# tungphambasement/TNN

Hardware: AMD Instinct MI355X
Metric: images/sec (whole node) WRN-16-8 on 32x32x3, pipeline-parallel (higher is better)
Workload: dtype bf16; 1 GPU; model=cifar100_wrn16_8, global_batch=256, input=32x32x3, microbatches=1, graphed_step=True, parallelism=single

## Files before the change

tnn_amd/csrc/batchnorm.hip:

```cpp

#include "common.h"
#include "kernels.h"

namespace tnn {

template <typename T> struct alignas(16) BnPack {
  T e[16 / sizeof(T)];
};

template <typename T>
__global__ void k_bn_partial(const T* __restrict__ x, float* __restrict__ sum,
                             float* __restrict__ sumsq, int64_t rows,
                             int cols) {
  const int cpb = min(cols, 256);
  const int rows_per_iter = 256 / cpb;
  const int c = threadIdx.x % cpb + blockIdx.x * cpb;
  const int r_off = threadIdx.x / cpb;
  if (c >= cols || r_off >= rows_per_iter) return;
  const int64_t r0 = rows * blockIdx.y / gridDim.y;
  const int64_t r1 = rows * (blockIdx.y + 1) / gridDim.y;
  const float k = VecIO<T>::to_f32(x[c]);
  float s = 0.0f, ss = 0.0f;
  for (int64_t r = r0 + r_off; r < r1; r += rows_per_iter) {
    float v = VecIO<T>::to_f32(x[r * cols + c]) - k;
// ... 62 lines not shown
      ts += sh_s[(r * gpb + gl) * V + j];
      tss += sh_ss[(r * gpb + gl) * V + j];
    }
    int c = blockIdx.x * cpb_total + cl;
    if (c >= cols) break;
    sum[(int64_t)blockIdx.y * 2 * cols + c] = ts;
    sum[(int64_t)blockIdx.y * 2 * cols + cols + c] = tss;
  }
}

template <typename T>
__global__ void k_bn_bwd_reduce_vec(const T* __restrict__ x,
                                    const T* __restrict__ dy,
                                    const T* __restrict__ y_relu,
                                    const float* mean, const float* invstd,
                                    float* __restrict__ sum_dy,
                                    float* __restrict__ sum_dy_xhat,
                                    int64_t rows, int cols, float dy_scale) {
  constexpr int V = 16 / sizeof(T);
  using VecT = BnPack<T>;
  const int groups = cols / V;
  const int gpb = min(groups, 256);
  const int rows_per_iter = 256 / gpb;
  const int g = threadIdx.x % gpb + blockIdx.x * gpb;
  const int r_off = threadIdx.x / gpb;
  __shared__ float sh[2 * 256 * V];
  float* sh_s = sh;
  float* sh_sx = sh + 256 * V;
  float s[V] = {}, sx[V] = {};
  if (g < groups && r_off < rows_per_iter) {
    const int64_t r0 = rows * blockIdx.y / gridDim.y;
    const int64_t r1 = rows * (blockIdx.y + 1) / gridDim.y;
    float m[V], is[V];
#pragma unroll
    for (int j = 0; j < V; ++j) {
      m[j] = mean[g * V + j];
      is[j] = invstd[g * V + j];
    }
#pragma unroll 2
    for (int64_t r = r0 + r_off; r < r1; r += rows_per_iter) {
      int64_t i = r * cols + (int64_t)g * V;
      VecT vg = *(const VecT*)&dy[i];
      VecT vx = *(const VecT*)&x[i];
      if (y_relu) {
        VecT vy = *(const VecT*)&y_relu[i];
#pragma unroll
        for (int j = 0; j < V; ++j) {
          float gr = VecIO<T>::to_f32(vy.e[j]) > 0.0f
                         ? VecIO<T>::to_f32(vg.e[j]) * dy_scale : 0.0f;
          s[j] += gr;
          sx[j] += gr * (VecIO<T>::to_f32(vx.e[j]) - m[j]) * is[j];
        }
      } else {
#pragma unroll
        for (int j = 0; j < V; ++j) {
          float gr = VecIO<T>::to_f32(vg.e[j]) * dy_scale;
          s[j] += gr;
          sx[j] += gr * (VecIO<T>::to_f32(vx.e[j]) - m[j]) * is[j];
        }
      }
    }
  }
#pragma unroll
  for (int j = 0; j < V; ++j) {
    sh_s[threadIdx.x * V + j] = s[j];
    sh_sx[threadIdx.x * V + j] = sx[j];
  }
  __syncthreads();
  const int cpb_total = gpb * V;
  for (int cl = threadIdx.x; cl < cpb_total; cl += 256) {
    int gl = cl / V, j = cl % V;
    float ts = 0.0f, tsx = 0.0f;
    for (int r = 0; r < rows_per_iter; ++r) {
      ts += sh_s[(r * gpb + gl) * V + j];
      tsx += sh_sx[(r * gpb + gl) * V + j];
    }
    int c = blockIdx.x * cpb_total + cl;
    if (c >= cols) break;
    sum_dy[(int64_t)blockIdx.y * 2 * cols + c] = ts;
    sum_dy[(int64_t)blockIdx.y * 2 * cols + cols + c] = tsx;
  }
}

template <typename T>
__global__ void k_bn_finalize(float* mean, float* invstd, const float* sum,
                              const float* sumsq, const T* shift, float* rmean,
                              float* rvar, float momentum, int64_t rows,
                              int cols, float eps) {
  int c = blockIdx.x * blockDim.x + threadIdx.x;
  if (c >= cols) return;
  float d = sum[c] / rows;
  float var = fmaxf(sumsq[c] / rows - d * d, 0.0f);
  float m = shift ? VecIO<T>::to_f32(shift[c]) + d : d;
  mean[c] = m;
  invstd[c] = rsqrtf(var + eps);
  if (rmean) {
    float unbiased = var * ((float)rows / (float)(rows > 1 ? rows - 1 : 1));
    rmean[c] = rmean[c] * (1.0f - momentum) + m * momentum;
    rvar[c] = rvar[c] * (1.0f - momentum) + unbiased * momentum;
  }
}

template <typename T>
__global__ void k_bn_apply(const T* __restrict__ x, const float* mean,
                           const float* invstd, const float* gamma,
                           const float* beta, T* __restrict__ y, int64_t n,
                           int cols, bool relu) {
  int64_t i = (int64_t)blockIdx.x * blockDim.x + threadIdx.x;
  int64_t stride = (int64_t)gridDim.x * blockDim.x;
  for (; i < n; i += stride) {
    int c = i % cols;
    float v = (VecIO<T>::to_f32(x[i]) - mean[c]) * invstd[c] * gamma[c] + beta[c];
    if (relu) v = fmaxf(v, 0.0f);
    y[i] = VecIO<T>::from_f32(v);
  }
}

template <typename T>
__global__ void k_bn_apply_drop(const T* __restrict__ x, const float* mean,
                                const float* invstd, const float* gamma,
                                const float* beta, T* __restrict__ y,
                                int64_t n, int cols, float p, uint64_t seed,
                                const int64_t* __restrict__ ctr) {
  if (ctr) seed ^= (uint64_t)(*ctr) * 0x9E3779B97F4A7C15ull;
  const float scale = 1.0f / (1.0f - p);
  Philox rng(seed);
  int64_t i4 = (int64_t)blockIdx.x * blockDim.x + threadIdx.x;
  int64_t stride = (int64_t)gridDim.x * blockDim.x;
  for (; i4 * 4 < n; i4 += stride) {
    uint4 r = rng(i4);
    unsigned int rs[4] = {r.x, r.y, r.z, r.w};
#pragma unroll
    for (int j = 0; j < 4; ++j) {
      int64_t i = i4 * 4 + j;
      if (i < n) {
        int c = i % cols;
        float v =
            (VecIO<T>::to_f32(x[i]) - mean[c]) * invstd[c] * gamma[c] + beta[c];
        v = fmaxf(v, 0.0f);
        bool keep = u32_to_uniform(rs[j]) > p;
        y[i] = VecIO<T>::from_f32(keep ? v * scale : 0.0f);
      }
    }
  }
}

template <typename T>
__global__ void k_bn_apply_drop_vec(const T* __restrict__ x, const float* mean,
                                    const float* invstd, const float* gamma,
                                    const float* beta, T* __restrict__ y,
                                    int64_t nv, int groups, float p,
                                    uint64_t seed,
                                    const int64_t* __restrict__ ctr) {
  if (ctr) seed ^= (uint64_t)(*ctr) * 0x9E3779B97F4A7C15ull;
  constexpr int V = 16 / sizeof(T);
  using VecT = BnPack<T>;
  const float scale = 1.0f / (1.0f - p);
  Philox rng(seed);
  int64_t i = (int64_t)blockIdx.x * blockDim.x + threadIdx.x;
  int64_t stride = (int64_t)gridDim.x * blockDim.x;
  for (; i < nv; i += stride) {
    int c0 = (int)((uint32_t)i % (uint32_t)groups) * V;
    VecT vx = ((const VecT*)x)[i];
    uint4 r0 = rng(2 * i);
    uint4 r1 = rng(2 * i + 1);
    unsigned int rs[8] = {r0.x, r0.y, r0.z, r0.w, r1.x, r1.y, r1.z, r1.w};
    VecT vy;
#pragma unroll
    for (int j = 0; j < V; ++j) {
      int c = c0 + j;
      float v =
          (VecIO<T>::to_f32(vx.e[j]) - mean[c]) * invstd[c] * gamma[c] + beta[c];
      v = fmaxf(v, 0.0f);
      bool keep = u32_to_uniform(rs[j]) > p;
      vy.e[j] = VecIO<T>::from_f32(keep ? v * scale : 0.0f);
    }
    ((VecT*)y)[i] = vy;
  }
}

template <typename T>
__global__ void k_bn_infer(const T* __restrict__ x, const float* rmean,
                           const float* rvar, const float* gamma,
// ... 148 lines not shown
  int cblocks = (groups + gpb - 1) / gpb;
  int rows_per_iter = 256 / gpb;
  int64_t iters = (rows + rows_per_iter - 1) / rows_per_iter;
  int rslices = (int)std::min<int64_t>(std::max<int64_t>(512 / cblocks, 1),
                                       std::max<int64_t>(iters / 4, 1));
  return dim3(cblocks, rslices);
}

static inline dim3 bn_reduce_grid(int64_t rows, int cols) {
  int cpb = cols < 256 ? cols : 256;
  int cblocks = (cols + cpb - 1) / cpb;
  int rows_per_iter = 256 / cpb;
  int64_t iters = (rows + rows_per_iter - 1) / rows_per_iter;
  int rslices = (int)std::min<int64_t>(std::max<int64_t>(512 / cblocks, 1),
                                       std::max<int64_t>(iters / 4, 1));
  return dim3(cblocks, rslices);
}

int64_t bn_stats_ws_floats(DT dt, const void* x, int64_t rows, int cols) {
  const bool vec = dt == DT::F32 ? bn_vec_ok<float>((void*)x, cols)
                                 : bn_vec_ok<bf16>((void*)x, cols);
  if (!vec) return 0;
  dim3 g = dt == DT::F32 ? bn_reduce_grid_vec<float>(rows, cols)
                         : bn_reduce_grid_vec<bf16>(rows, cols);
  return ((int64_t)g.y + 1) * 2 * cols;
}

void bn_stats_launch(DT dt, const void* x, float* mean, float* invstd,
                     float* rmean, float* rvar, float momentum, float* ws,
                     int64_t rows, int cols, float eps, hipStream_t s) {
  if (ws) {
    dim3 g = dt == DT::F32 ? bn_reduce_grid_vec<float>(rows, cols)
                           : bn_reduce_grid_vec<bf16>(rows, cols);
    float* sums = ws + (int64_t)g.y * 2 * cols;
    if (dt == DT::F32)
      hipLaunchKernelGGL(k_bn_partial_vec<float>, g, dim3(256), 0, s,
                         (const float*)x, ws, nullptr, rows, cols);
    else
      hipLaunchKernelGGL(k_bn_partial_vec<bf16>, g, dim3(256), 0, s,
                         (const bf16*)x, ws, nullptr, rows, cols);
    slab_fin_launch(ws, sums, (int)g.y, 2 * cols, s);
    if (dt == DT::F32)
      hipLaunchKernelGGL(k_bn_finalize<float>, dim3((cols + 255) / 256),
                         dim3(256), 0, s, mean, invstd, sums, sums + cols,
                         (const float*)x, rmean, rvar, momentum, rows, cols,
                         eps);
    else
      hipLaunchKernelGGL(k_bn_finalize<bf16>, dim3((cols + 255) / 256),
                         dim3(256), 0, s, mean, invstd, sums, sums + cols,
                         (const bf16*)x, rmean, rvar, momentum, rows, cols,
                         eps);
    return;
  }
  hipMemsetAsync(mean, 0, cols * sizeof(float), s);
  hipMemsetAsync(invstd, 0, cols * sizeof(float), s);
  if (dt == DT::F32)
    hipLaunchKernelGGL(k_bn_partial<float>, bn_reduce_grid(rows, cols),
                       dim3(256), 0, s, (const float*)x, mean, invstd, rows,
                       cols);
  else
    hipLaunchKernelGGL(k_bn_partial<bf16>, bn_reduce_grid(rows, cols),
                       dim3(256), 0, s, (const bf16*)x, mean, invstd, rows,
                       cols);
  if (dt == DT::F32)
    hipLaunchKernelGGL(k_bn_finalize<float>, dim3((cols + 255) / 256),
                       dim3(256), 0, s, mean, invstd, mean, invstd,
                       (const float*)x, rmean, rvar, momentum, rows, cols, eps);
  else
    hipLaunchKernelGGL(k_bn_finalize<bf16>, dim3((cols + 255) / 256),
                       dim3(256), 0, s, mean, invstd, mean, invstd,
                       (const bf16*)x, rmean, rvar, momentum, rows, cols, eps);
}

void bn_finalize_launch(const float* sum, const float* sumsq, float* mean,
                        float* invstd, float* rmean, float* rvar,
                        float momentum, int64_t rows, int cols, float eps,
                        hipStream_t s) {
  hipLaunchKernelGGL(k_bn_finalize<float>, dim3((cols + 255) / 256),
                     dim3(256), 0, s, mean, invstd, sum, sumsq,
                     (const float*)nullptr, rmean, rvar, momentum, rows, cols,
                     eps);
}

void bn_apply_launch(DT dt, const void* x, const float* mean,
                     const float* invstd, const float* gamma, const float* beta,
                     void* y, int64_t rows, int cols, bool relu,
                     hipStream_t s) {
  int64_t n = rows * cols;
  int blocks = (int)std::min<int64_t>((n + 255) / 256, (int64_t)2048);
  if (dt == DT::F32) {
    if (bn_vec_ok<float>(x, cols)) {
      hipLaunchKernelGGL(k_bn_apply_vec<float>, dim3(blocks), dim3(256), 0, s,
                         (const float*)x, mean, invstd, gamma, beta, (float*)y,
                         n / 4, cols / 4, relu);
      return;
    }
    hipLaunchKernelGGL(k_bn_apply<float>, dim3(blocks), dim3(256), 0, s,
                       (const float*)x, mean, invstd, gamma, beta, (float*)y, n,
                       cols, relu);
  } else {
    if (bn_vec_ok<bf16>(x, cols)) {
      hipLaunchKernelGGL(k_bn_apply_vec<bf16>, dim3(blocks), dim3(256), 0, s,
                         (const bf16*)x, mean, invstd, gamma, beta, (bf16*)y,
                         n / 8, cols / 8, relu);
      return;
    }
    hipLaunchKernelGGL(k_bn_apply<bf16>, dim3(blocks), dim3(256), 0, s,
                       (const bf16*)x, mean, invstd, gamma, beta, (bf16*)y, n,
                       cols, relu);
  }
}

void bn_apply_drop_launch(DT dt, const void* x, const float* mean,
                          const float* invstd, const float* gamma,
                          const float* beta, void* y, int64_t rows, int cols,
                          float p, uint64_t seed, const int64_t* ctr,
                          hipStream_t s) {
  int64_t n = rows * cols;
  int V = dt == DT::F32 ? 4 : 8;
  if (cols % V == 0 && (((uintptr_t)x & 15) == 0) && n < (1ll << 34)) {
    int64_t nv = n / V;
    int blocks = (int)std::min<int64_t>((nv + 255) / 256, (int64_t)2048);
    if (dt == DT::F32)
      hipLaunchKernelGGL(k_bn_apply_drop_vec<float>, dim3(blocks), dim3(256),
                         0, s, (const float*)x, mean, invstd, gamma, beta,
                         (float*)y, nv, cols / V, p, seed, ctr);
    else
      hipLaunchKernelGGL(k_bn_apply_drop_vec<bf16>, dim3(blocks), dim3(256),
                         0, s, (const bf16*)x, mean, invstd, gamma, beta,
                         (bf16*)y, nv, cols / V, p, seed, ctr);
    return;
  }
  int blocks = (int)std::min<int64_t>(((n + 3) / 4 + 255) / 256, (int64_t)2048);
  if (dt == DT::F32)
    hipLaunchKernelGGL(k_bn_apply_drop<float>, dim3(blocks), dim3(256), 0, s,
                       (const float*)x, mean, invstd, gamma, beta, (float*)y, n,
                       cols, p, seed, ctr);
  else
    hipLaunchKernelGGL(k_bn_apply_drop<bf16>, dim3(blocks), dim3(256), 0, s,
                       (const bf16*)x, mean, invstd, gamma, beta, (bf16*)y, n,
                       cols, p, seed, ctr);
}

void bn_infer_launch(DT dt, const void* x, const float* rmean,
                     const float* rvar, const float* gamma, const float* beta,
                     void* y, int64_t rows, int cols, float eps, bool relu,
                     hipStream_t s) {
  int64_t n = rows * cols;
  int blocks = (int)std::min<int64_t>((n + 255) / 256, (int64_t)2048);
  if (dt == DT::F32)
    hipLaunchKernelGGL(k_bn_infer<float>, dim3(blocks), dim3(256), 0, s,
                       (const float*)x, rmean, rvar, gamma, beta, (float*)y, n,
                       cols, eps, relu);
  else
    hipLaunchKernelGGL(k_bn_infer<bf16>, dim3(blocks), dim3(256), 0, s,
                       (const bf16*)x, rmean, rvar, gamma, beta, (bf16*)y, n,
                       cols, eps, relu);
}

int64_t bn_bwd_ws_floats(DT dt, const void* x, const void* dy, int64_t rows,
                         int cols) {
  const bool vec = dt == DT::F32
                       ? (bn_vec_ok<float>((void*)x, cols) &&
                          bn_vec_ok<float>((void*)dy, cols))
                       : (bn_vec_ok<bf16>((void*)x, cols) &&
                          bn_vec_ok<bf16>((void*)dy, cols));
  if (!vec) return 0;
  dim3 g = dt == DT::F32 ? bn_reduce_grid_vec<float>(rows, cols)
                         : bn_reduce_grid_vec<bf16>(rows, cols);
  return (int64_t)g.y * 2 * cols;
}

void bn_bwd_reduce_launch(DT dt, const void* x, const void* dy,
                          const void* y_relu, const float* mean,
                          const float* invstd, float* sum_dy,
                          float* sum_dy_xhat, float* ws, int64_t rows,
                          int cols, float dy_scale, hipStream_t s) {
  if (ws) {
    dim3 g = dt == DT::F32 ? bn_reduce_grid_vec<float>(rows, cols)
                           : bn_reduce_grid_vec<bf16>(rows, cols);
    if (dt == DT::F32)
      hipLaunchKernelGGL(k_bn_bwd_reduce_vec<float>, g, dim3(256), 0, s,
                         (const float*)x, (const float*)dy,
                         (const float*)y_relu, mean, invstd, ws, nullptr,
                         rows, cols, dy_scale);
    else
      hipLaunchKernelGGL(k_bn_bwd_reduce_vec<bf16>, g, dim3(256), 0, s,
                         (const bf16*)x, (const bf16*)dy, (const bf16*)y_relu,
                         mean, invstd, ws, nullptr, rows, cols, dy_scale);
    slab_fin_launch(ws, sum_dy, (int)g.y, 2 * cols, s);
    return;
  }
  if (dt == DT::F32)
    hipLaunchKernelGGL(k_bn_bwd_reduce<float>, bn_reduce_grid(rows, cols),
                       dim3(256), 0, s, (const float*)x, (const float*)dy,
                       (const float*)y_relu, mean, invstd, sum_dy,
                       sum_dy_xhat, rows, cols, dy_scale);
  else
    hipLaunchKernelGGL(k_bn_bwd_reduce<bf16>, bn_reduce_grid(rows, cols),
                       dim3(256), 0, s, (const bf16*)x, (const bf16*)dy,
                       (const bf16*)y_relu, mean, invstd, sum_dy,
                       sum_dy_xhat, rows, cols, dy_scale);
}

void bn_bwd_apply_launch(DT dt, const void* x, const void* dy,
                         const void* y_relu, const float* mean,
                         const float* invstd, const float* gamma,
                         const float* sum_dy, const float* sum_dy_xhat,
                         void* dx, const void* resid, int64_t rows, int cols,
                         float dy_scale, hipStream_t s) {
  int64_t n = rows * cols;
  int blocks = (int)std::min<int64_t>((n + 255) / 256, (int64_t)2048);
  const bool vec = dt == DT::F32 ? bn_vec_ok<float>(x, cols)
                                 : bn_vec_ok<bf16>(x, cols);
  if (dt == DT::F32) {
    if (vec && ((uintptr_t)dy & 15) == 0) {
      hipLaunchKernelGGL(k_bn_bwd_apply_vec<float>, dim3(blocks), dim3(256),
                         0, s, (const float*)x, (const float*)dy,
                         (const float*)y_relu, mean, invstd, gamma, sum_dy,
                         sum_dy_xhat, (float*)dx, (const float*)resid,
                         n / 4, cols / 4, rows, dy_scale);
      return;
    }
    hipLaunchKernelGGL(k_bn_bwd_apply<float>, dim3(blocks), dim3(256), 0, s,
                       (const float*)x, (const float*)dy, (const float*)y_relu,
                       mean, invstd, gamma, sum_dy, sum_dy_xhat, (float*)dx,
                       (const float*)resid, n, rows, cols, dy_scale);
  } else {
    if (vec && ((uintptr_t)dy & 15) == 0) {
      hipLaunchKernelGGL(k_bn_bwd_apply_vec<bf16>, dim3(blocks), dim3(256),
                         0, s, (const bf16*)x, (const bf16*)dy,
                         (const bf16*)y_relu, mean, invstd, gamma, sum_dy,
                         sum_dy_xhat, (bf16*)dx, (const bf16*)resid,
                         n / 8, cols / 8, rows, dy_scale);
      return;
    }
    hipLaunchKernelGGL(k_bn_bwd_apply<bf16>, dim3(blocks), dim3(256), 0, s,
                       (const bf16*)x, (const bf16*)dy, (const bf16*)y_relu,
                       mean, invstd, gamma, sum_dy, sum_dy_xhat, (bf16*)dx,
                       (const bf16*)resid, n, rows, cols, dy_scale);
  }
}

}
```

tnn_amd/csrc/bindings.cpp:

```cpp

#include <array>
#include <torch/extension.h>
#include <ATen/hip/HIPContext.h>

#include "kernels.h"

namespace tnn {

static hipStream_t cur_stream() {
  return at::hip::getCurrentHIPStreamMasqueradingAsCUDA().stream();
}

static void* zero_page(const at::Tensor& like) {
  static at::Tensor z;
  if (!z.defined() || z.device() != like.device())
    z = at::zeros({16}, like.options().dtype(at::kFloat));
  return z.data_ptr();
}

static DT dt_of(const at::Tensor& t) {
  if (t.scalar_type() == at::kFloat) return DT::F32;
  if (t.scalar_type() == at::kBFloat16) return DT::BF16;
  TORCH_CHECK(false, "tnn_amd kernels support fp32/bf16, got ", t.scalar_type());
}
// ... 394 lines not shown
  int64_t H = x.size(1), W = x.size(2);
  return conv_shape_out(fn, x.size(0), H, W, Cin, Cout, KH, KW, SH, SW, PH, PW,
                        conv_out_extent(H, KH, SH, PH),
                        conv_out_extent(W, KW, SW, PW));
}

static ConvShape conv_fwd_shape(const char* fn, const at::Tensor& x,
                                const at::Tensor& w, int64_t sh, int64_t sw,
                                int64_t ph, int64_t pw) {
  CHECK_IN(x);
  CHECK_IN(w);
  TORCH_CHECK(x.dim() == 4 && w.dim() == 4 && x.size(3) == w.size(2), fn,
              " x ", x.sizes(), " w ", w.sizes());
  TORCH_CHECK(x.scalar_type() == w.scalar_type(), fn, " dtype mismatch ",
              x.scalar_type(), " vs ", w.scalar_type());
  return conv_shape(fn, x, w.size(2), w.size(3), w.size(0), w.size(1), sh, sw,
                    ph, pw);
}

static ConvShape conv_dgrad_shape(const char* fn, const at::Tensor& dy,
                                  const at::Tensor& w, int64_t H, int64_t W,
                                  int64_t sh, int64_t sw, int64_t ph,
                                  int64_t pw) {
  CHECK_IN(dy);
  CHECK_IN(w);
  TORCH_CHECK(dy.dim() == 4 && w.dim() == 4, fn, " dy ", dy.sizes(), " w ",
              w.sizes());
  TORCH_CHECK(dy.scalar_type() == w.scalar_type(), fn,
              " dtype mismatch: dy is ", dy.scalar_type(), ", w is ",
              w.scalar_type());
  TORCH_CHECK(dy.size(3) == w.size(3), fn, " dy ", dy.sizes(),
              " has other channels than w ", w.sizes());
  const int64_t KH = w.size(0), KW = w.size(1);
  auto cs = conv_shape_out(fn, dy.size(0), H, W, w.size(2), w.size(3), KH, KW,
                           sh, sw, ph, pw, conv_out_extent(H, KH, sh, ph),
                           conv_out_extent(W, KW, sw, pw));
  TORCH_CHECK(dy.size(1) == cs.OH && dy.size(2) == cs.OW, fn, " dy ",
              dy.sizes(), " is not the output of a ", H, " x ", W,
              " input: expected OH = ", cs.OH, ", OW = ", cs.OW);
  return cs;
}

static ConvShape conv_wgrad_shape(const char* fn, const at::Tensor& x,
                                  const at::Tensor& dy, int64_t KH, int64_t KW,
                                  int64_t sh, int64_t sw, int64_t ph,
                                  int64_t pw) {
  CHECK_IN(x);
  CHECK_IN(dy);
  TORCH_CHECK(x.dim() == 4 && dy.dim() == 4, fn, " x ", x.sizes(), " dy ",
              dy.sizes());
  TORCH_CHECK(x.scalar_type() == dy.scalar_type(), fn,
              " dtype mismatch: x is ", x.scalar_type(), ", dy is ",
              dy.scalar_type());
  TORCH_CHECK(x.size(0) == dy.size(0), fn, " batch mismatch: x ", x.sizes(),
              " dy ", dy.sizes());
  auto cs = conv_shape(fn, x, x.size(3), dy.size(3), KH, KW, sh, sw, ph, pw);
  TORCH_CHECK(dy.size(1) == cs.OH && dy.size(2) == cs.OW, "wgrad shape");
  return cs;
}

static std::vector<at::Tensor> conv2d_fwd_impl(
    const at::Tensor& x, const at::Tensor& w,
    const c10::optional<at::Tensor>& bias, int64_t sh, int64_t sw, int64_t ph,
    int64_t pw, bool relu, bool want_stats) {
  auto cs = conv_fwd_shape("conv2d_fwd", x, w, sh, sw, ph, pw);
  if (bias.has_value()) {
    TORCH_CHECK(bias->scalar_type() == x.scalar_type(),
                "conv2d bias dtype mismatch");
    TORCH_CHECK(bias->is_cuda() && bias->is_contiguous() &&
                    bias->numel() == cs.Cout,
                "conv2d_fwd: bias must be a contiguous GPU tensor of ",
                cs.Cout, " elements, got ", bias->sizes());
  }
  auto y = at::empty({cs.N, cs.OH, cs.OW, cs.Cout}, x.options());
  at::Tensor wt2, stats;
  const bool db = conv2d_fwd_wants_db(dt_of(x), x.data_ptr(), cs);
  if (db) {
    wt2 = at::empty({(int64_t)cs.Cout, (int64_t)cs.KH * cs.KW * cs.Cin},
                    w.options());
    transpose_w_fwd_launch(dt_of(x), w.data_ptr(), wt2.data_ptr(),
                           cs.KH * cs.KW, cs.Cin, cs.Cout, cur_stream());
  }
  if (want_stats)
    stats = db ? at::zeros({2, (int64_t)cs.Cout},
                           x.options().dtype(at::kFloat))
               : at::empty({0}, x.options().dtype(at::kFloat));
  conv2d_fwd_launch(dt_of(x), x.data_ptr(), w.data_ptr(),
                    db ? wt2.data_ptr() : nullptr,
                    bias.has_value() ? bias->data_ptr() : nullptr,
                    y.data_ptr(), zero_page(x),
                    db && want_stats ? stats.data_ptr<float>() : nullptr, cs,
                    relu, cur_stream());
  return {y, stats};
}

at::Tensor conv2d_fwd(const at::Tensor& x, const at::Tensor& w,
                      const c10::optional<at::Tensor>& bias, int64_t sh,
                      int64_t sw, int64_t ph, int64_t pw, bool relu) {
  return conv2d_fwd_impl(x, w, bias, sh, sw, ph, pw, relu, false)[0];
}

std::vector<at::Tensor> conv2d_fwd_stats(const at::Tensor& x,
                                         const at::Tensor& w,
                                         const c10::optional<at::Tensor>& bias,
                                         int64_t sh, int64_t sw, int64_t ph,
                                         int64_t pw) {
  return conv2d_fwd_impl(x, w, bias, sh, sw, ph, pw, false, true);
}

at::Tensor conv2d_dgrad(const at::Tensor& dy, const at::Tensor& w, int64_t H,
                        int64_t W, int64_t sh, int64_t sw, int64_t ph,
                        int64_t pw) {
  auto cs = conv_dgrad_shape("conv2d_dgrad", dy, w, H, W, sh, sw, ph, pw);
  int KH = cs.KH, KW = cs.KW, Cin = cs.Cin, Cout = cs.Cout;
  auto dx = at::empty({cs.N, H, W, Cin}, dy.options());
  if (conv2d_dgrad_wants_db(dt_of(dy), dy.data_ptr(), cs)) {
    auto w_t2d = at::empty({Cin, (int64_t)KH * KW * Cout}, w.options());
    transpose_w_dgrad_launch(dt_of(w), w.data_ptr(), w_t2d.data_ptr(), KH * KW,
                             Cin, Cout, cur_stream());
    conv2d_dgrad_launch(dt_of(dy), dy.data_ptr(), nullptr, w_t2d.data_ptr(),
                        dx.data_ptr(), zero_page(dy), cs, cur_stream());
    return dx;
  }
  auto w_t = at::empty({KH, KW, Cout, Cin}, w.options());
  transpose_w_launch(dt_of(w), w.data_ptr(), w_t.data_ptr(), KH, KW, Cin, Cout,
                     cur_stream());
  conv2d_dgrad_launch(dt_of(dy), dy.data_ptr(), w_t.data_ptr(), nullptr,
                      dx.data_ptr(), zero_page(dy), cs, cur_stream());
  return dx;
}

std::string conv2d_fwd_route_name(const at::Tensor& x, const at::Tensor& w,
                                  int64_t sh, int64_t sw, int64_t ph,
                                  int64_t pw, bool stats) {
  auto cs = conv_fwd_shape("conv2d_fwd_route", x, w, sh, sw, ph, pw);
  return conv2d_fwd_route(dt_of(x), x.data_ptr(), cs, stats);
}

std::string conv2d_dgrad_route_name(const at::Tensor& dy,
                                    const at::Tensor& w, int64_t H, int64_t W,
                                    int64_t sh, int64_t sw, int64_t ph,
                                    int64_t pw) {
  auto cs = conv_dgrad_shape("conv2d_dgrad_route", dy, w, H, W, sh, sw, ph,
                             pw);
  return conv2d_dgrad_route(dt_of(dy), dy.data_ptr(), cs);
}

std::tuple<std::string, int64_t> conv2d_wgrad_route_name(
    const at::Tensor& x, const at::Tensor& dy, int64_t KH, int64_t KW,
    int64_t sh, int64_t sw, int64_t ph, int64_t pw) {
  auto cs = conv_wgrad_shape("conv2d_wgrad_route", x, dy, KH, KW, sh, sw, ph,
                             pw);
  return {conv2d_wgrad_route(dt_of(x), x.data_ptr(), dy.data_ptr(), cs),
          conv2d_wgrad_zsplits(dt_of(x), x.data_ptr(), dy.data_ptr(), cs)};
}

static at::Tensor conv2d_wgrad_rows(const at::Tensor& x, const at::Tensor& dy,
                                    int64_t KH, int64_t KW, int64_t sh,
                                    int64_t sw, int64_t ph, int64_t pw,
                                    bool out_in_dt, bool bias) {
  auto cs = conv_wgrad_shape("conv2d_wgrad", x, dy, KH, KW, sh, sw, ph, pw);
  DT out_dt = out_in_dt ? dt_of(x) : DT::F32;
  const int64_t rows = KH * KW * cs.Cin + (bias ? 1 : 0);
  auto out = at::empty({rows, (int64_t)cs.Cout},
                       out_dt == DT::F32 ? x.options().dtype(at::kFloat)
                                         : x.options());
  int z = conv2d_wgrad_zsplits(dt_of(x), x.data_ptr(), dy.data_ptr(), cs);
  at::Tensor ws;
  float* wsp = nullptr;
  if (z > 1 || out_dt != DT::F32) {
    ws = at::empty({(int64_t)z * rows * cs.Cout},
                   x.options().dtype(at::kFloat));
    wsp = ws.data_ptr<float>();
  }
  conv2d_wgrad_launch(dt_of(x), x.data_ptr(), dy.data_ptr(), out.data_ptr(),
                      out_dt, wsp, z, zero_page(x), cs, bias, cur_stream());
  return out;
}

at::Tensor conv2d_wgrad(const at::Tensor& x, const at::Tensor& dy, int64_t KH,
                        int64_t KW, int64_t sh, int64_t sw, int64_t ph,
                        int64_t pw, bool out_in_dt) {
  return conv2d_wgrad_rows(x, dy, KH, KW, sh, sw, ph, pw, out_in_dt, false)
      .view({KH, KW, x.size(3), dy.size(3)});
}

std::vector<at::Tensor> conv2d_wgrad_bias(const at::Tensor& x,
                                          const at::Tensor& dy, int64_t KH,
                                          int64_t KW, int64_t sh, int64_t sw,
                                          int64_t ph, int64_t pw,
                                          bool out_in_dt) {
  auto out = conv2d_wgrad_rows(x, dy, KH, KW, sh, sw, ph, pw, out_in_dt, true);
  const int64_t kout = out.size(0) - 1;
  return {out.narrow(0, 0, kout).view({KH, KW, x.size(3), dy.size(3)}),
          out.select(0, kout)};
}

std::vector<at::Tensor> bn_fwd_train(const at::Tensor& x,
                                     const at::Tensor& gamma,
                                     const at::Tensor& beta,
                                     const c10::optional<at::Tensor>& rmean,
                                     const c10::optional<at::Tensor>& rvar,
                                     double momentum, double eps, bool relu,
                                     double dropout_p, int64_t seed,
                                     const c10::optional<at::Tensor>& precomp,
                                     const c10::optional<at::Tensor>& ctr =
                                         c10::nullopt) {
  CHECK_IN(x);
  TORCH_CHECK(dropout_p == 0.0 || relu, "fused BN dropout requires relu");
  int C = x.size(-1);
  int64_t rows = x.numel() / C;
  auto mean = at::empty({C}, x.options().dtype(at::kFloat));
  auto invstd = at::empty({C}, x.options().dtype(at::kFloat));
  auto y = at::empty_like(x);
  float* rm = rmean.has_value() ? rmean->data_ptr<float>() : nullptr;
  float* rv = rvar.has_value() ? rvar->data_ptr<float>() : nullptr;
  if (precomp.has_value()) {
    TORCH_CHECK(precomp->numel() == 2 * C, "bad precomputed stats");
    const float* ps = precomp->data_ptr<float>();
    bn_finalize_launch(ps, ps + C, mean.data_ptr<float>(),
                       invstd.data_ptr<float>(), rm, rv, (float)momentum,
                       rows, C, (float)eps, cur_stream());
  } else {
    const int64_t wsn = bn_stats_ws_floats(dt_of(x), x.data_ptr(), rows, C);
    at::Tensor ws;
    float* wp = nullptr;
    if (wsn) {
      ws = at::empty({wsn}, x.options().dtype(at::kFloat));
      wp = ws.data_ptr<float>();
    }
    bn_stats_launch(dt_of(x), x.data_ptr(), mean.data_ptr<float>(),
                    invstd.data_ptr<float>(), rm, rv, (float)momentum, wp,
                    rows, C, (float)eps, cur_stream());
  }
  if (dropout_p > 0.0)
    bn_apply_drop_launch(dt_of(x), x.data_ptr(), mean.data_ptr<float>(),
                         invstd.data_ptr<float>(), gamma.data_ptr<float>(),
                         beta.data_ptr<float>(), y.data_ptr(), rows, C,
                         (float)dropout_p, (uint64_t)seed,
                         ctr.has_value() ? ctr->data_ptr<int64_t>() : nullptr,
                         cur_stream());
  else
    bn_apply_launch(dt_of(x), x.data_ptr(), mean.data_ptr<float>(),
                    invstd.data_ptr<float>(), gamma.data_ptr<float>(),
                    beta.data_ptr<float>(), y.data_ptr(), rows, C, relu,
                    cur_stream());
  return {y, mean, invstd};
}

at::Tensor bn_fwd_infer(const at::Tensor& x, const at::Tensor& gamma,
                        const at::Tensor& beta, const at::Tensor& rmean,
                        const at::Tensor& rvar, double eps, bool relu) {
  CHECK_IN(x);
  int C = x.size(-1);
  int64_t rows = x.numel() / C;
  auto y = at::empty_like(x);
  bn_infer_launch(dt_of(x), x.data_ptr(), rmean.data_ptr<float>(),
                  rvar.data_ptr<float>(), gamma.data_ptr<float>(),
                  beta.data_ptr<float>(), y.data_ptr(), rows, C, (float)eps,
                  relu, cur_stream());
  return y;
}

std::vector<at::Tensor> bn_bwd(const at::Tensor& x, const at::Tensor& dy,
                               const at::Tensor& gamma, const at::Tensor& mean,
                               const at::Tensor& invstd,
                               const c10::optional<at::Tensor>& y_relu,
                               double dy_scale,
                               const c10::optional<at::Tensor>& resid =
                                   c10::nullopt) {
  CHECK_IN(x);
  CHECK_IN(dy);
  const void* resp = nullptr;
  if (resid.has_value()) {
    TORCH_CHECK(resid->is_contiguous() &&
                resid->scalar_type() == x.scalar_type() &&
                resid->numel() == x.numel(), "bn_bwd resid mismatch");
    resp = resid->data_ptr();
  }
  int C = x.size(-1);
  int64_t rows = x.numel() / C;
  const int64_t wsn = bn_bwd_ws_floats(dt_of(x), x.data_ptr(),
                                       dy.data_ptr(), rows, C);
  auto sums = wsn ? at::empty({2, C}, x.options().dtype(at::kFloat))
                  : at::zeros({2, C}, x.options().dtype(at::kFloat));
  auto sum_dy = sums[0];
  auto sum_dy_xhat = sums[1];
  at::Tensor ws;
  float* wp = nullptr;
  if (wsn) {
    ws = at::empty({wsn}, x.options().dtype(at::kFloat));
    wp = ws.data_ptr<float>();
  }
  auto dx = at::empty_like(x);
  const void* yr = y_relu.has_value() ? y_relu->data_ptr() : nullptr;
  bn_bwd_reduce_launch(dt_of(x), x.data_ptr(), dy.data_ptr(), yr,
                       mean.data_ptr<float>(), invstd.data_ptr<float>(),
                       sum_dy.data_ptr<float>(), sum_dy_xhat.data_ptr<float>(),
                       wp, rows, C, (float)dy_scale, cur_stream());
  bn_bwd_apply_launch(dt_of(x), x.data_ptr(), dy.data_ptr(), yr,
                      mean.data_ptr<float>(), invstd.data_ptr<float>(),
                      gamma.data_ptr<float>(), sum_dy.data_ptr<float>(),
                      sum_dy_xhat.data_ptr<float>(), dx.data_ptr(), resp,
                      rows, C, (float)dy_scale, cur_stream());
  return {dx, sum_dy_xhat, sum_dy};
}

static PoolShape pool_shape(const at::Tensor& x, int KH, int KW, int SH, int SW,
                            int PH, int PW) {
  PoolShape ps;
  ps.N = x.size(0);
  ps.H = x.size(1);
  ps.W = x.size(2);
  ps.C = x.size(3);
  ps.KH = KH;
  ps.KW = KW;
  ps.SH = SH;
  ps.SW = SW;
  ps.PH = PH;
  ps.PW = PW;
  ps.OH = (ps.H + 2 * PH - KH) / SH + 1;
  ps.OW = (ps.W + 2 * PW - KW) / SW + 1;
  return ps;
}

std::vector<at::Tensor> maxpool_fwd(const at::Tensor& x, int64_t kh, int64_t kw,
                                    int64_t sh, int64_t sw, int64_t ph,
                                    int64_t pw) {
  CHECK_IN(x);
  auto ps = pool_shape(x, kh, kw, sh, sw, ph, pw);
  auto y = at::empty({ps.N, ps.OH, ps.OW, ps.C}, x.options());
  auto idx = at::empty({ps.N, ps.OH, ps.OW, ps.C}, x.options().dtype(at::kInt));
  maxpool_fwd_launch(dt_of(x), x.data_ptr(), y.data_ptr(), idx.data_ptr<int>(),
                     ps, cur_stream());
  return {y, idx};
}

at::Tensor maxpool_bwd(const at::Tensor& dy, const at::Tensor& idx, int64_t H,
                       int64_t W) {
  CHECK_IN(dy);
  PoolShape ps;
  ps.N = dy.size(0);
  ps.OH = dy.size(1);
  ps.OW = dy.size(2);
  ps.C = dy.size(3);
  ps.H = H;
  ps.W = W;
  auto dxf = at::zeros({ps.N, H, W, ps.C}, dy.options().dtype(at::kFloat));
  maxpool_bwd_launch(dt_of(dy), dy.data_ptr(), idx.data_ptr<int>(),
                     dxf.data_ptr<float>(), ps, cur_stream());
  if (dy.scalar_type() == at::kFloat) return dxf;
  auto dx = at::empty({ps.N, H, W, ps.C}, dy.options());
  cast_f32_launch(dt_of(dy), dxf.data_ptr<float>(), dx.data_ptr(), dx.numel(),
                  cur_stream());
  return dx;
}

at::Tensor avgpool_fwd(const at::Tensor& x, int64_t kh, int64_t kw, int64_t sh,
                       int64_t sw, int64_t ph, int64_t pw) {
  CHECK_IN(x);
  auto ps = pool_shape(x, kh, kw, sh, sw, ph, pw);
  auto y = at::empty({ps.N, ps.OH, ps.OW, ps.C}, x.options());
  avgpool_fwd_launch(dt_of(x), x.data_ptr(), y.data_ptr(), ps, cur_stream());
  return y;
}

at::Tensor avgpool_bwd(const at::Tensor& dy, int64_t H, int64_t W, int64_t kh,
                       int64_t kw, int64_t sh, int64_t sw, int64_t ph,
                       int64_t pw) {
  CHECK_IN(dy);
  PoolShape ps;
  ps.N = dy.size(0);
  ps.OH = dy.size(1);
  ps.OW = dy.size(2);
  ps.C = dy.size(3);
  ps.H = H;
  ps.W = W;
  ps.KH = kh;
  ps.KW = kw;
  ps.SH = sh;
  ps.SW = sw;
  ps.PH = ph;
  ps.PW = pw;
  auto dx = at::empty({ps.N, H, W, ps.C}, dy.options());
  avgpool_bwd_launch(dt_of(dy), dy.data_ptr(), dx.data_ptr(), ps, cur_stream());
  return dx;
}

// ... 577 lines not shown
                cap = k_cache.size(2), D = k_cache.size(3);
  const int64_t T = k_new.size(2);
  const int64_t per = 16 / k_cache.element_size();
  auto vec_ok = [&](const at::Tensor& t) {
    return ((uintptr_t)t.data_ptr() & 15) == 0 && t.stride(0) % per == 0 &&
           t.stride(1) % per == 0 && t.stride(2) % per == 0;
  };
  const bool vec = D % per == 0 && vec_ok(k_new) && vec_ok(v_new) &&
                   vec_ok(k_cache) && vec_ok(v_cache);
  const std::array<int64_t, 3> ks = {k_new.stride(0), k_new.stride(1),
                                     k_new.stride(2)};
  const std::array<int64_t, 3> vs = {v_new.stride(0), v_new.stride(1),
                                     v_new.stride(2)};
  kv_append_n_launch(dt, k_cache.data_ptr(), v_cache.data_ptr(),
                     k_new.data_ptr(), v_new.data_ptr(),
                     pos.data_ptr<int64_t>(),
                     n_new.has_value() ? n_new->data_ptr<int64_t>() : nullptr,
                     (int)B, (int)H, (int)T, (int)cap, (int)D, ks.data(),
                     vs.data(), vec, cur_stream());
}

at::Tensor sample_logits(const at::Tensor& logits, double temperature,
                         int64_t top_k, double top_p, int64_t seed,
                         const at::Tensor& step,
                         const c10::optional<at::Tensor>& u) {
  CHECK_IN(logits);
  TORCH_CHECK(logits.dim() == 2 && logits.scalar_type() == at::kBFloat16,
              "sample_logits wants bf16 [R,V] logits");
  const int64_t R = logits.size(0), V = logits.size(1);
  TORCH_CHECK(V >= 1 && V < (int64_t)1 << 31, "sample_logits: bad V ", V);
  TORCH_CHECK(temperature >= 0.0 && top_k >= 0 && top_p > 0.0 && top_p <= 1.0,
              "sample_logits wants temperature >= 0, top_k >= 0, top_p in "
              "(0, 1]");
  TORCH_CHECK(step.is_cuda() && step.scalar_type() == at::kLong &&
              step.numel() == 1, "sample_logits step must be int64 [1]");
  const float* up = nullptr;
  if (u.has_value()) {
    TORCH_CHECK(u->is_cuda() && u->is_contiguous() &&
                u->scalar_type() == at::kFloat && u->numel() == R,
                "sample_logits u must be fp32 [R] on device");
    up = u->data_ptr<float>();
  }
  auto ids = at::empty({R}, logits.options().dtype(at::kLong));
  if (R > 0)
    sample_logits_launch(logits.data_ptr(), ids.data_ptr<int64_t>(), (int)R,
                         (int)V, (float)temperature,
                         (int)std::min<int64_t>(top_k, V), (float)top_p,
                         (uint64_t)seed, step.data_ptr<int64_t>(), up,
                         cur_stream());
  return ids;
}

namespace imgcodec {
at::Tensor decode_image(const py::bytes& data);
}

}

PYBIND11_MODULE(TORCH_EXTENSION_NAME, m) {
  m.def("act_fwd", &tnn::act_fwd);
  m.def("act_bwd", &tnn::act_bwd);
  m.def("relu_bwd_mask", &tnn::relu_bwd_mask);
  m.def("add_act_fwd", &tnn::add_act_fwd);
  m.def("add_act_bwd", &tnn::add_act_bwd);
  m.def("dropout_fwd", &tnn::dropout_fwd, py::arg("x"), py::arg("p"),
        py::arg("seed"), py::arg("ctr") = c10::nullopt);
  m.def("dropout_bwd", &tnn::dropout_bwd);
  m.def("colsum", &tnn::colsum);
  m.def("gemm", &tnn::gemm, py::arg("a"), py::arg("b"), py::arg("bias"),
        py::arg("act_kind"), py::arg("residual") = c10::nullopt,
        py::arg("ln_gamma") = c10::nullopt, py::arg("ln_beta") = c10::nullopt,
        py::arg("ln_eps") = 1e-5);
  m.def("gemm_skinny", &tnn::gemm_skinny, py::arg("a"), py::arg("b"),
        py::arg("bias"), py::arg("act_kind"),
        py::arg("residual") = c10::nullopt, py::arg("ln_gamma") = c10::nullopt,
        py::arg("ln_beta") = c10::nullopt, py::arg("ln_eps") = 1e-5);
  m.def("skinny_enabled", &tnn::skinny_enabled);
  m.def("gemm_nt", &tnn::gemm_nt);
  m.def("gemm_tn", &tnn::gemm_tn);
  m.def("mfma_selftest", &tnn::mfma_selftest);
  m.def("mfma_selftest_f32", &tnn::mfma_selftest_f32);
  m.def("conv2d_fwd", &tnn::conv2d_fwd);
  m.def("conv2d_fwd_stats", &tnn::conv2d_fwd_stats);
  m.def("conv2d_dgrad", &tnn::conv2d_dgrad);
  m.def("conv2d_fwd_route", &tnn::conv2d_fwd_route_name);
  m.def("conv2d_dgrad_route", &tnn::conv2d_dgrad_route_name);
  m.def("conv2d_wgrad_route", &tnn::conv2d_wgrad_route_name);
  m.def("conv2d_wgrad", &tnn::conv2d_wgrad);
  m.def("conv2d_wgrad_bias", &tnn::conv2d_wgrad_bias);
  m.def("bn_fwd_train", &tnn::bn_fwd_train, py::arg("x"), py::arg("gamma"),
        py::arg("beta"), py::arg("rmean"), py::arg("rvar"),
        py::arg("momentum"), py::arg("eps"), py::arg("relu"),
        py::arg("dropout_p"), py::arg("seed"), py::arg("precomp"),
        py::arg("ctr") = c10::nullopt);
  m.def("bn_fwd_infer", &tnn::bn_fwd_infer);
  m.def("bn_bwd", &tnn::bn_bwd, py::arg("x"), py::arg("dy"),
        py::arg("gamma"), py::arg("mean"), py::arg("invstd"),
        py::arg("y_relu"), py::arg("dy_scale"),
        py::arg("resid") = py::none());
  m.def("maxpool_fwd", &tnn::maxpool_fwd);
  m.def("maxpool_bwd", &tnn::maxpool_bwd);
  m.def("avgpool_fwd", &tnn::avgpool_fwd);
  m.def("avgpool_bwd", &tnn::avgpool_bwd);
  m.def("ce_fwd", &tnn::ce_fwd);
  m.def("ce_bwd", &tnn::ce_bwd);
  m.def("ptloss_fwd", &tnn::ptloss_fwd);
  m.def("ptloss_bwd", &tnn::ptloss_bwd);
  m.def("gn_fwd", &tnn::gn_fwd);
  m.def("gn_bwd", &tnn::gn_bwd);
  m.def("ln_fwd", &tnn::ln_fwd);
  m.def("ln_bwd", &tnn::ln_bwd, py::arg("x"), py::arg("dy"),
        py::arg("gamma"), py::arg("mean"), py::arg("invstd"),
        py::arg("resid") = py::none());
  m.def("embedding_fwd", &tnn::embedding_fwd);
  m.def("embedding_bwd", &tnn::embedding_bwd);
  m.def("attn_fwd", &tnn::attn_fwd);
  m.def("attn_bwd", &tnn::attn_bwd, py::arg("q"), py::arg("k"),
        py::arg("v"), py::arg("o"), py::arg("dout"), py::arg("lse"),
        py::arg("causal"), py::arg("dq_out") = py::none(),
        py::arg("dk_out") = py::none(), py::arg("dv_out") = py::none());
  m.def("bmm", &tnn::bmm);
  m.def("smax_fwd", &tnn::smax_fwd);
  m.def("smax_bwd", &tnn::smax_bwd);
  m.def("attn_decode", &tnn::attn_decode);
  m.def("kv_append", &tnn::kv_append);
  m.def("attn_extend", &tnn::attn_extend);
  m.def("kv_append_n", &tnn::kv_append_n);
  m.def("sample_logits", &tnn::sample_logits, py::arg("logits"),
        py::arg("temperature"), py::arg("top_k"), py::arg("top_p"),
        py::arg("seed"), py::arg("step"), py::arg("u") = c10::nullopt);
  m.def("sgd_step", &tnn::sgd_step, py::arg("param"), py::arg("master"),
        py::arg("grad"), py::arg("momentum_buf"), py::arg("lr"),
        py::arg("momentum"), py::arg("weight_decay"), py::arg("nesterov"),
        py::arg("clip") = c10::nullopt, py::arg("lr_dev") = c10::nullopt);
  m.def("adam_step", &tnn::adam_step, py::arg("param"), py::arg("master"),
        py::arg("grad"), py::arg("m"), py::arg("v"), py::arg("step"),
        py::arg("lr"), py::arg("beta1"), py::arg("beta2"), py::arg("eps"),
        py::arg("weight_decay"), py::arg("adamw"),
        py::arg("step_dev") = c10::nullopt, py::arg("clip") = c10::nullopt,
        py::arg("lr_dev") = c10::nullopt);
  m.def("adam_step_mt", &tnn::adam_step_mt, py::arg("desc"),
        py::arg("chunks"), py::arg("dt_p"), py::arg("dt_g"),
        py::arg("has_master"), py::arg("step"), py::arg("lr"),
        py::arg("beta1"), py::arg("beta2"), py::arg("eps"),
        py::arg("weight_decay"), py::arg("adamw"),
        py::arg("step_dev") = c10::nullopt, py::arg("clip") = c10::nullopt,
        py::arg("lr_dev") = c10::nullopt);
  m.def("grad_sumsq_mt", &tnn::grad_sumsq_mt, py::arg("desc"),
        py::arg("chunks"), py::arg("stride"), py::arg("gslot"),
        py::arg("nslot"), py::arg("dt_g"), py::arg("part"), py::arg("base"));
  m.def("clip_finalize", &tnn::clip_finalize, py::arg("part"),
        py::arg("npart"), py::arg("max_norm"), py::arg("state"),
        py::arg("skipped") = c10::nullopt, py::arg("sumsq_in") = c10::nullopt);
  m.def("decode_image", &tnn::imgcodec::decode_image);
}
```

tnn_amd/csrc/conv2d.hip:

```cpp

#include "common.h"
#include "kernels.h"
#include "tile_gemm.h"

namespace tnn {

using namespace tile;

template <bool POW2>
DEV int idiv(int x, const IDiv& f) {
  if constexpr (POW2) return x >> f.lg;
  else if (f.magic)
    return (int)(((unsigned long long)(unsigned)x * f.magic) >> f.sh);
  else
    return x / f.d;
}
template <bool POW2>
DEV int imod(int x, const IDiv& f) {
  if constexpr (POW2) return x & (f.d - 1);
  else return x - idiv<POW2>(x, f) * f.d;
}

DEV void kdecode(int kidx, const ConvShape& cs, int& kh, int& kw) {
  kh = (kidx * cs.mkw16) >> 16;
// ... 89 lines not shown
    int rem = row - n * (Hc * Wc);
    ih = idiv<POW2>(rem, cs.d_w);
    iw = rem - ih * Wc;
    if constexpr (S2) {
      ih = 2 * ih + cls_a;
      iw = 2 * iw + cls_b;
    }
  }
  template <bool POW2>
  DEV int64_t pixel(const ConvShape& cs, int row) const {
    if constexpr (!S2) return row;
    int n, ih, iw;
    coords<POW2>(cs, row, n, ih, iw);
    return ((int64_t)n * cs.H + ih) * cs.W + iw;
  }
};
template <bool S2, bool S1, typename T>
DEV const T* dgrad_src(const T* __restrict__ DY, const ConvShape& cs, int n,
                       int ih, int iw, int kh, int kw, int co, const T* oob) {
  int th = ih + cs.PH - kh, tw = iw + cs.PW - kw;
  int oh, ow;
  if constexpr (S2) {
    if (th < 0 || tw < 0) return oob;
    oh = th >> 1, ow = tw >> 1;
    if (oh >= cs.OH || ow >= cs.OW) return oob;
  } else if constexpr (S1) {
    if (th < 0 || tw < 0 || th >= cs.OH || tw >= cs.OW) return oob;
    oh = th, ow = tw;
  } else {
    if (th < 0 || tw < 0 || th % cs.SH || tw % cs.SW) return oob;
    oh = th / cs.SH, ow = tw / cs.SW;
    if (oh >= cs.OH || ow >= cs.OW) return oob;
  }
  return &DY[(((int64_t)n * cs.OH + oh) * cs.OW + ow) * cs.Cout + co];
}

template <typename T, typename GatherFn>
DEV void stage_a_gathered(T* As, int m0, int k0, int M, int K,
                          GatherFn&& gather) {
  constexpr int V = 16 / sizeof(T);
#pragma unroll
  for (int c = threadIdx.x; c < BM * (BK / V); c += THREADS) {
    int row = c / (BK / V);
    int kk = (c % (BK / V)) * V;
    int gm = m0 + row, gk = k0 + kk;
    Pack16<T> v = {};
    if (gm < M && gk < K) v = gather(gm, gk);
    *(Pack16<T>*)&As[lds_off<T>(row, kk)] = v;
  }
}
template <typename T, typename RowFn>
DEV void stage_b_transposed(T* Bs, RowFn&& rowptr, int ncols, int n0, int k0,
                            int K) {
  constexpr int V = 16 / sizeof(T);
#pragma unroll
  for (int c = threadIdx.x; c < BK * (BN / V); c += THREADS) {
    int kk = c / (BN / V);
    int nn = (c % (BN / V)) * V;
    int gk = k0 + kk;
    Pack16<T> v = {};
    if (gk < K) v = load16_guarded(rowptr(gk), n0 + nn, ncols);
#pragma unroll
    for (int j = 0; j < V; ++j)
      Bs[lds_off<T>(nn + j, kk)] = v.e[j];
  }
}


template <typename T, typename S>
DEV void conv_fwd_store(const WaveCoordT<S>& wc, f32x4 acc[S::FM][S::FN],
                        const T* bias, T* Y, const ConvShape& cs, int act_kind,
                        int m0, int n0, int M) {
  epilogue_visit(wc, acc, m0, n0, [&](int row, int col, float v) {
    if (row < M && col < cs.Cout) {
      if (bias) v += VecIO<T>::to_f32(bias[col]);
      if (act_kind != ACT_LINEAR) v = act_apply(v, act_kind);
      Y[(int64_t)row * cs.Cout + col] = VecIO<T>::from_f32(v);
    }
  });
}

template <typename T, typename S>
DEV void conv_fwd_stats(const WaveCoordT<S>& wc, f32x4 acc[S::FM][S::FN],
                        const T* bias_p, float* stats, const ConvShape& cs,
                        int m0, int n0, int M) {
  constexpr int FM = S::FM, FN = S::FN;
  float* ssum = stats;
  float* ssumsq = stats + cs.Cout;
  const int cr = (wc.lane >> 4) * 4;
  const int cc = wc.lane & 15;
#pragma unroll
  for (int fn = 0; fn < FN; ++fn) {
    int col = n0 + wc.wcol0 + fn * 16 + cc;
    float bias = 0.0f;
    if (col < cs.Cout) {
      if (bias_p) bias = VecIO<T>::to_f32(bias_p[col]);
    }
    float s = 0.0f, ss = 0.0f;
#pragma unroll
    for (int fm = 0; fm < FM; ++fm)
#pragma unroll
      for (int j = 0; j < 4; ++j) {
        int row = m0 + wc.wrow0 + fm * 16 + cr + j;
        if (row < M && col < cs.Cout) {
          float v = acc[fm][fn][j] + bias;
          s += v;
          ss += v * v;
        }
      }
    s += __shfl_xor(s, 16, 64);
    ss += __shfl_xor(ss, 16, 64);
    s += __shfl_xor(s, 32, 64);
    ss += __shfl_xor(ss, 32, 64);
    if (wc.lane < 16 && col < cs.Cout) {
      atomicAdd(&ssum[col], s);
      atomicAdd(&ssumsq[col], ss);
    }
  }
}

template <bool POW2, typename T, bool S2, typename S>
DEV void dgrad_store(const WaveCoordT<S>& wc, f32x4 acc[S::FM][S::FN], T* DX,
                     const ConvShape& cs, const DgradClass<S2>& dc, int m0,
                     int n0) {
  epilogue_visit(wc, acc, m0, n0, [&](int row, int col, float v) {
    if (row < dc.M && col < cs.Cin)
      DX[dc.template pixel<POW2>(cs, row) * cs.Cin + col] =
          VecIO<T>::from_f32(v);
  });
}

template <typename S>
DEV float* wgrad_slab_store(const WaveCoordT<S>& wc,
                            f32x4 acc[S::FM][S::FN], float* DW,
                            const ConvShape& cs, int Kout, int bias_row,
                            int r0, int n0) {
  float* out = DW + (int64_t)blockIdx.z * (Kout + bias_row) * cs.Cout;
  epilogue_visit(wc, acc, r0, n0, [&](int row, int col, float v) {
    if (row < Kout && col < cs.Cout) out[(int64_t)row * cs.Cout + col] = v;
  });
  return out;
}
template <typename S>
DEV void wgrad_biasrow_store(float* out, const WaveCoordT<S>& wc,
                             const f32x4 (&bacc)[S::FN / S::WAVES_M],
                             const ConvShape& cs, int Kout, int n0) {
  constexpr int NBF = S::FN / S::WAVES_M;
  const int wm = wc.wid / S::WAVES_N;
  if (wc.lane < 16) {
#pragma unroll
    for (int t = 0; t < NBF; ++t) {
      int col = n0 + wc.wcol0 + 16 * (NBF * wm + t) + wc.lane;
      if (col < cs.Cout) out[(int64_t)Kout * cs.Cout + col] = bacc[t][0];
    }
  }
}
DEV void wgrad_colsum_store(float* out, const ConvShape& cs, int Kout, int n0,
                            float bsum) {
  bsum = colsum_tile_finish(bsum);
  int col = n0 + (threadIdx.x >> 2);
  if ((threadIdx.x & 3) == 0 && col < cs.Cout)
    out[(int64_t)Kout * cs.Cout + col] = bsum;
}

template <bool DB, typename T, typename S, typename RowFn, typename TapFn,
          typename AtFn>
DEV void conv_db_kloop(T* As0, T* As1, T* Bs0, T* Bs1,
                       const WaveCoordT<S>& wc, f32x4 acc[S::FM][S::FN],
                       const T* __restrict__ asrc, int lgSW, int lgC,
                       const T* __restrict__ bsrc, int64_t bstride,
                       int brows, int m0, int n0, int K,
                       const T* __restrict__ zero16, RowFn&& row,
                       TapFn&& tap, AtFn&& at) {
  constexpr int NA = glds_count<T, S::BM>();
  constexpr int NB = glds_count<T, S::BN>();
  constexpr int NPER = NA + NB;
  const int wid = __builtin_amdgcn_readfirstlane(wc.wid);
  const bool uni = lgC >= 6;

  const T* ab[NA];
  int ap[NA], aq[NA];
  const T* bb[NB];
  bool bok[NB];
#pragma unroll
  for (int i = 0; i < NA; ++i) {
    const int j = wid * NA + i;
    int64_t noff;
    int p, q;
    const bool ok = row(m0 + glds_row<T>(j, wc.lane), noff, p, q);
    ab[i] = asrc + noff + (uni ? glds_kk<T>(j, wc.lane) : 0);
    ap[i] = ok ? p : -(1 << 28);
    aq[i] = q;
  }
#pragma unroll
  for (int i = 0; i < NB; ++i) {
    const int j = wid * NB + i;
    const int gn = n0 + glds_row<T>(j, wc.lane);
    bok[i] = gn < brows;
    bb[i] = bsrc + (int64_t)gn * bstride + (uni ? glds_kk<T>(j, wc.lane) : 0);
  }
// ... 43 lines not shown
  const int nch = (K + BK - 1) / BK;
  if (nch == 0) return;
  auto compute = [&](const T* a_img, const T* b_img) {
    if constexpr (sizeof(T) == 2)
      mfma_compute_tile_nofence(a_img, b_img, wc, acc);
    else
      mfma_compute_tile(a_img, b_img, wc, acc);
  };
  auto step = [&](int t, T* a_cur, T* b_cur, T* a_nxt, T* b_nxt) {
    if (t + 1 < nch) {
      stage(t + 1, a_nxt, b_nxt);
      wait_vmcnt<NPER>();
    } else {
      wait_vmcnt<0>();
    }
    __builtin_amdgcn_s_barrier();
    compute(a_cur, b_cur);
    __builtin_amdgcn_s_barrier();
  };
  if constexpr (DB) {
    stage(0, As0, Bs0);
    for (int t = 0; t < nch; t += 2) {
      step(t, As0, Bs0, As1, Bs1);
      if (t + 1 < nch) step(t + 1, As1, Bs1, As0, Bs0);
    }
  } else {
    for (int t = 0; t < nch; ++t) {
      stage(t, As0, Bs0);
      wait_vmcnt<0>();
      __builtin_amdgcn_s_barrier();
      compute(As0, Bs0);
      __builtin_amdgcn_s_barrier();
    }
  }
}

template <typename T, bool STATS, bool DB, typename S = TileStd>
DEV void conv_fwd_glds_tile(const T* __restrict__ X,
                            const T* __restrict__ WT2,
                            const T* __restrict__ bias, T* __restrict__ Y,
                            const T* __restrict__ zero16, const ConvShape& cs,
                            int act_kind, float* __restrict__ stats) {
  const int M = cs.N * cs.OH * cs.OW;
  const int K = cs.KH * cs.KW * cs.Cin;
  int tm_, tn_;
  conv_tile_order(cs, tm_, tn_);
  const int m0 = tm_ * S::BM;
  const int n0 = tn_ * S::BN;
  const WaveCoordT<S> wc;
  f32x4 acc[S::FM][S::FN] = {};

  auto row = [&](int gm, int64_t& noff, int& p, int& q) {
    const int n = gm >> cs.d_ohow.lg;
    const int rem = gm & (cs.OH * cs.OW - 1);
    p = (rem >> cs.d_ow.lg) * cs.SH - cs.PH;
    q = (rem & (cs.OW - 1)) * cs.SW - cs.PW;
    noff = (int64_t)n << (cs.d_hw.lg + cs.d_cin.lg);
    return gm < M;
  };
  auto tap = [&](int gk, int& dh, int& dw, int& c, int& bcol) {
    kdecode(gk >> cs.d_cin.lg, cs, dh, dw);
    c = gk & (cs.Cin - 1);
    bcol = gk;
  };
  auto at = [&](int p, int q, int dh, int dw, int& ih, int& iw) {
    ih = p + dh;
    iw = q + dw;
    return (unsigned)ih < (unsigned)cs.H && (unsigned)iw < (unsigned)cs.W;
  };
  if constexpr (DB) {
    __shared__ alignas(16) T As0[S::BM * BK], As1[S::BM * BK];
    __shared__ alignas(16) T Bs0[S::BN * BK], Bs1[S::BN * BK];
    conv_db_kloop<true>(As0, As1, Bs0, Bs1, wc, acc, X, cs.d_w.lg,
                        cs.d_cin.lg, WT2, (int64_t)K, cs.Cout, m0, n0, K,
                        zero16, row, tap, at);
  } else {
    __shared__ alignas(16) T As0[S::BM * BK], Bs0[S::BN * BK];
    conv_db_kloop<false>(As0, As0, Bs0, Bs0, wc, acc, X, cs.d_w.lg,
                         cs.d_cin.lg, WT2, (int64_t)K, cs.Cout, m0, n0, K,
                         zero16, row, tap, at);
  }

  conv_fwd_store(wc, acc, bias, Y, cs, act_kind, m0, n0, M);
  if constexpr (STATS) conv_fwd_stats(wc, acc, bias, stats, cs, m0, n0, M);
}

template <typename T, bool STATS = false>
__launch_bounds__(THREADS)
__global__ void k_conv_fwd_db(const T* __restrict__ X,
                              const T* __restrict__ WT2,
                              const T* __restrict__ bias, T* __restrict__ Y,
                              const T* __restrict__ zero16, ConvShape cs,
                              int act_kind, float* __restrict__ stats) {
  conv_fwd_glds_tile<T, STATS, true>(X, WT2, bias, Y, zero16, cs, act_kind,
                                     stats);
}

template <bool STATS>
__launch_bounds__(THREADS)
__global__ void k_conv_fwd_sb(const bf16* __restrict__ X,
                              const bf16* __restrict__ WT2,
                              const bf16* __restrict__ bias,
                              bf16* __restrict__ Y,
                              const bf16* __restrict__ zero16, ConvShape cs,
                              int act_kind, float* __restrict__ stats) {
  conv_fwd_glds_tile<bf16, STATS, false>(X, WT2, bias, Y, zero16, cs, act_kind,
                                         stats);
}

template <bool STATS>
__launch_bounds__(THREADS, 2)
__global__ void k_conv_fwd_db_wide(const bf16* __restrict__ X,
                                   const bf16* __restrict__ WT2,
                                   const bf16* __restrict__ bias,
                                   bf16* __restrict__ Y,
                                   const bf16* __restrict__ zero16,
                                   ConvShape cs, int act_kind,
                                   float* __restrict__ stats) {
  conv_fwd_glds_tile<bf16, STATS, true, TileWide>(X, WT2, bias, Y, zero16, cs,
                                                  act_kind, stats);
}
template <bool STATS>
__launch_bounds__(THREADS, 3)
__global__ void k_conv_fwd_sb_wide(const bf16* __restrict__ X,
                                   const bf16* __restrict__ WT2,
                                   const bf16* __restrict__ bias,
                                   bf16* __restrict__ Y,
                                   const bf16* __restrict__ zero16,
                                   ConvShape cs, int act_kind,
                                   float* __restrict__ stats) {
  conv_fwd_glds_tile<bf16, STATS, false, TileWide>(X, WT2, bias, Y, zero16, cs,
                                                   act_kind, stats);
}

template <typename T, bool POW2, bool GLDS>
__launch_bounds__(THREADS)
__global__ void k_conv_fwd(const T* __restrict__ X, const T* __restrict__ Wt,
                           const T* __restrict__ bias, T* __restrict__ Y,
                           const T* __restrict__ zero16, ConvShape cs,
                           int act_kind) {
  static_assert(!GLDS || POW2, "the LDS-DMA gate implies an all-pow2 shape");
  __shared__ alignas(16) T As[BM * BK];
  __shared__ alignas(16) T Bs[BN * BK];

  const int M = cs.N * cs.OH * cs.OW;
  const int K = cs.KH * cs.KW * cs.Cin;
  int tm_, tn_;
  conv_tile_order(cs, tm_, tn_);
  const int m0 = tm_ * BM;
  const int n0 = tn_ * BN;
  const WaveCoord wc;
  f32x4 acc[FM][FN] = {};

  auto a_src = [&](int k0, int rl, int kk) -> const T* {
    int gm = m0 + rl, gk = k0 + kk;
    if (gm >= M || gk >= K) return zero16;
    return fwd_src<POW2>(X, cs, fwd_row<POW2>(cs, gm), gk, zero16);
  };

  for (int k0 = 0; k0 < K; k0 += BK) {
    if constexpr (GLDS) {
      glds_stage_a<T>(As, wc, [&](int rl, int kk) { return a_src(k0, rl, kk); });
    } else {
      stage_a_gathered(As, m0, k0, M, K, [&](int gm, int gk) {
        return fwd_gather16<POW2>(X, cs, fwd_row<POW2>(cs, gm), gk, K);
      });
    }
// ... 462 lines not shown
                                    T* __restrict__ out, int rows, int cols) {
  __shared__ T tile[32][33];
  const int c0 = blockIdx.x * 32, r0 = blockIdx.y * 32;
  const int64_t slice = (int64_t)blockIdx.z * rows * cols;
  const T* src = in + slice;
  T* dst = out + slice;
  const int tx = threadIdx.x & 31, ty = threadIdx.x >> 5;
#pragma unroll
  for (int d = 0; d < 32; d += 8) {
    int r = r0 + ty + d, c = c0 + tx;
    if (r < rows && c < cols) tile[ty + d][tx] = src[(int64_t)r * cols + c];
  }
  __syncthreads();
#pragma unroll
  for (int d = 0; d < 32; d += 8) {
    int c = c0 + ty + d, r = r0 + tx;
    if (c < cols && r < rows) dst[(int64_t)c * rows + r] = tile[tx][ty + d];
  }
}

template <typename T>
__global__ void k_transpose_w_dgrad(const T* __restrict__ W,
                                    T* __restrict__ WT2D, int KHW, int Cin,
                                    int Cout) {
  int64_t i = (int64_t)blockIdx.x * blockDim.x + threadIdx.x;
  int64_t n = (int64_t)KHW * Cin * Cout;
  if (i >= n) return;
  int co = i % Cout;
  int ci = (i / Cout) % Cin;
  int64_t khw = i / ((int64_t)Cin * Cout);
  WT2D[((int64_t)ci * KHW + khw) * Cout + co] = W[i];
}

template <typename T>
__global__ void k_transpose_w_dgrad_vec(const T* __restrict__ W,
                                        T* __restrict__ WT2D, int KHW,
                                        int Cin, int Cout) {
  constexpr int V = 16 / sizeof(T);
  struct alignas(16) P { T e[16 / sizeof(T)]; };
  const int cov = Cout / V;
  int64_t i = (int64_t)blockIdx.x * blockDim.x + threadIdx.x;
  int64_t n = (int64_t)KHW * Cin * cov;
  if (i >= n) return;
  int c = i % cov;
  int ci = (i / cov) % Cin;
  int64_t khw = i / ((int64_t)Cin * cov);
  ((P*)WT2D)[((int64_t)ci * KHW + khw) * cov + c] =
      ((const P*)W)[((int64_t)khw * Cin + ci) * cov + c];
}

static bool all_pow2(const ConvShape& cs) {
  return cs.d_ohow.lg >= 0 && cs.d_ow.lg >= 0 && cs.d_cin.lg >= 0 &&
         cs.d_hw.lg >= 0 && cs.d_w.lg >= 0 && cs.d_cout.lg >= 0;
}

static bool vec_ok(DT dt, const void* ptr, int channels) {
  return channels % vec_elems(dt) == 0 && ptr_aligned16(ptr);
}

static int env_int(const char* name, int dflt) {
  const char* e = getenv(name);
  return e ? atoi(e) : dflt;
}

static bool db_on() {
  static const bool on = env_int("TNN_FWD_DB", 1) != 0;
  return on;
}

static int fwd_db_maxk() {
  static const int maxk = env_int("TNN_DB_MAXK", 2304);
  return maxk;
}

static int wide_mode() {
  static const int mode = env_int("TNN_CONV_WIDE", 1);
  return mode;
}
static int wide_buf() {
  static const int buf = env_int("TNN_CONV_WIDE_BUF", 0);
  return buf;
}

enum class Wide { NO, DB, SB };
constexpr int WIDE_MIN_TILES = 512;
constexpr int WIDE_FWD_DB_MINK = 2048;
constexpr int WIDE_DGRAD_SB_MAXK = 1152;
static Wide wide_pick(bool eligible, int tiles, bool take, bool single) {
  if (!eligible || wide_mode() == 0) return Wide::NO;
  if (wide_mode() == 1 && !(take && tiles >= WIDE_MIN_TILES)) return Wide::NO;
  if (wide_buf() != 0) single = wide_buf() == 2;
  return single ? Wide::SB : Wide::DB;
}
static Wide fwd_wide(DT dt, bool have_wt2, const ConvShape& cs, bool stats) {
  const int nt = cs.Cout / TileWide::BN;
  const int K = cs.KH * cs.KW * cs.Cin;
  const bool take = nt == 1 ? !stats : K >= WIDE_FWD_DB_MINK;
  return wide_pick(
      have_wt2 && dt == DT::BF16 && cs.Cout % TileWide::BN == 0,
      ceil_div(cs.N * cs.OH * cs.OW, TileWide::BM) * nt, take, nt == 1);
}
static Wide dgrad_wide(DT dt, bool have_wt2d, bool s2, const ConvShape& cs) {
  const int M = s2 ? cs.N * (cs.H / 2) * (cs.W / 2) : cs.N * cs.H * cs.W;
  const int taps =
      s2 ? ((cs.KH + 1) / 2) * ((cs.KW + 1) / 2) : cs.KH * cs.KW;
  return wide_pick(
      have_wt2d && dt == DT::BF16 && cs.Cin % TileWide::BN == 0,
      ceil_div(M, TileWide::BM) * (cs.Cin / TileWide::BN) * (s2 ? 4 : 1),
      true, taps * cs.Cout <= WIDE_DGRAD_SB_MAXK);
}

template <typename... KArgs, typename... Args>
static void launch(void (*kern)(KArgs...), dim3 grid, hipStream_t s,
                   Args... args) {
  hipLaunchKernelGGL(kern, grid, dim3(THREADS), 0, s, args...);
}

bool conv2d_fwd_wants_db(DT dt, const void* x, const ConvShape& cs) {
  if (!db_on()) return false;
  if (dt == DT::F32 && cs.KH * cs.KW * cs.Cin > fwd_db_maxk()) return false;
  return all_pow2(cs) && vec_ok(dt, x, cs.Cin);
}

static void transpose2d_launch(DT dt, const void* in, void* out, int batch,
                               int rows, int cols, hipStream_t s) {
  dim3 grid((cols + 31) / 32, (rows + 31) / 32, batch);
  dispatch_dt(dt, [&](auto tag) {
    using T = typename decltype(tag)::type;
    hipLaunchKernelGGL(k_transpose2d_tiled<T>, grid, dim3(256), 0, s,
                       (const T*)in, (T*)out, rows, cols);
  });
}

void transpose_w_fwd_launch(DT dt, const void* w, void* w_t2, int KHW, int Cin,
                            int Cout, hipStream_t s) {
  transpose2d_launch(dt, w, w_t2, 1, KHW * Cin, Cout, s);
}

void transpose_w_launch(DT dt, const void* w, void* w_t, int KH, int KW,
                        int Cin, int Cout, hipStream_t s) {
  transpose2d_launch(dt, w, w_t, KH * KW, Cin, Cout, s);
}

void transpose_w_dgrad_launch(DT dt, const void* w, void* w_t2d, int KHW,
                              int Cin, int Cout, hipStream_t s) {
  const bool vec = vec_ok(dt, w, Cout);
  int64_t n = (int64_t)KHW * Cin * (vec ? Cout / vec_elems(dt) : Cout);
  int blocks = (int)((n + 255) / 256);
  dispatch_dt(dt, [&](auto tag) {
    using T = typename decltype(tag)::type;
    auto kern = vec ? k_transpose_w_dgrad_vec<T> : k_transpose_w_dgrad<T>;
    hipLaunchKernelGGL(kern, dim3(blocks), dim3(256), 0, s, (const T*)w,
                       (T*)w_t2d, KHW, Cin, Cout);
  });
}

enum class FwdRoute { SB_WIDE, DB_WIDE, SB, DB, GLDS, POW2, GENERIC };
static FwdRoute fwd_route(DT dt, const void* x, bool have_wt2,
                          const ConvShape& cs, bool stats) {
  if (have_wt2) {
    const Wide wide = fwd_wide(dt, true, cs, stats);
    if (wide != Wide::NO)
      return wide == Wide::SB ? FwdRoute::SB_WIDE : FwdRoute::DB_WIDE;
    const bool long_k =
        dt == DT::BF16 && cs.KH * cs.KW * cs.Cin > fwd_db_maxk();
    return long_k ? FwdRoute::SB : FwdRoute::DB;
  }
  if (!all_pow2(cs)) return FwdRoute::GENERIC;
  return vec_ok(dt, x, cs.Cin) ? FwdRoute::GLDS : FwdRoute::POW2;
}

const char* conv2d_fwd_route(DT dt, const void* x, const ConvShape& cs,
                             bool stats) {
  const bool db = conv2d_fwd_wants_db(dt, x, cs);
  switch (fwd_route(dt, x, db, cs, db && stats)) {
    case FwdRoute::SB_WIDE: return "k_conv_fwd_sb_wide";
    case FwdRoute::DB_WIDE: return "k_conv_fwd_db_wide";
    case FwdRoute::SB: return "k_conv_fwd_sb";
    case FwdRoute::DB: return "k_conv_fwd_db";
    case FwdRoute::GLDS: return "k_conv_fwd<pow2, glds>";
    case FwdRoute::POW2: return "k_conv_fwd<pow2>";
    default: return "k_conv_fwd";
  }
}

void conv2d_fwd_launch(DT dt, const void* x, const void* w, const void* w_t2,
                       const void* bias, void* y, const void* zero16,
                       float* stats, const ConvShape& cs, bool relu,
                       hipStream_t s) {
  int M = cs.N * cs.OH * cs.OW;
  dim3 grid(ceil_div(M, BM), ceil_div(cs.Cout, BN));
  dim3 grid_wide(ceil_div(M, TileWide::BM), ceil_div(cs.Cout, TileWide::BN));
  int act = relu ? ACT_RELU : ACT_LINEAR;
  const FwdRoute route =
      fwd_route(dt, x, w_t2 != nullptr, cs, stats != nullptr);
  dispatch_dt(dt, [&](auto tag) {
    using T = typename decltype(tag)::type;
    auto X = (const T*)x;
    auto B = (const T*)bias;
    auto Y = (T*)y;
    auto Z = (const T*)zero16;
    if constexpr (sizeof(T) == 2) {
      if (route == FwdRoute::SB_WIDE)
        return launch(
            stats ? k_conv_fwd_sb_wide<true> : k_conv_fwd_sb_wide<false>,
            grid_wide, s, X, (const T*)w_t2, B, Y, Z, cs, act, stats);
      if (route == FwdRoute::DB_WIDE)
        return launch(
            stats ? k_conv_fwd_db_wide<true> : k_conv_fwd_db_wide<false>,
            grid_wide, s, X, (const T*)w_t2, B, Y, Z, cs, act, stats);
      if (route == FwdRoute::SB)
        return launch(stats ? k_conv_fwd_sb<true> : k_conv_fwd_sb<false>,
                      grid, s, X, (const T*)w_t2, B, Y, Z, cs, act, stats);
    }
    if (route == FwdRoute::DB)
      return launch(stats ? k_conv_fwd_db<T, true> : k_conv_fwd_db<T, false>,
                    grid, s, X, (const T*)w_t2, B, Y, Z, cs, act, stats);
    launch(route == FwdRoute::GLDS
               ? k_conv_fwd<T, true, true>
               : (route == FwdRoute::POW2 ? k_conv_fwd<T, true, false>
                                          : k_conv_fwd<T, false, false>),
           grid, s, X, (const T*)w, B, Y, Z, cs, act);
  });
}

bool conv2d_dgrad_wants_db(DT dt, const void* dy, const ConvShape& cs) {
  if (!db_on()) return false;
  static const int maxk = env_int("TNN_DB_MAXK_DGRAD", 4608);
  return cs.KH * cs.KW * cs.Cout <= maxk && all_pow2(cs) &&
         vec_ok(dt, dy, cs.Cout);
}

static bool dgrad_parity(const ConvShape& cs, ConvShape& cs2) {
  bool s2 = all_pow2(cs) && cs.SH == 2 && cs.SW == 2 && cs.H % 2 == 0 &&
            cs.W % 2 == 0 && cs.KW <= 4;
  cs2 = cs;
  if (s2) {
    cs2.d_hw.set((cs.H / 2) * (cs.W / 2));
    cs2.d_w.set(cs.W / 2);
    s2 = cs2.d_hw.lg >= 0 && cs2.d_w.lg >= 0;
  }
  return s2;
}

// ... 87 lines not shown
}
static int wgrad_splits_pin() {
  static const int z = env_int("TNN_WGRAD_SPLITS", 0);
  return z;
}

enum class WgradRoute { TR_WIDE_DB, TR_WIDE_SB, TR, VEC, POW2, GENERIC };

constexpr int WGRAD_WIDE_WAVES = 1;
constexpr int WGRAD_WIDE_1TILE_MAXKOUT = 144;
constexpr int WGRAD_WIDE_SB_MINTILES = 144;
constexpr int WGRAD_WIDE_DB_SLOTS = 512, WGRAD_WIDE_SB_SLOTS = 768;
static int wgrad_wide_waves() {
  static const int n =
      std::max(env_int("TNN_WGRAD_WAVES", WGRAD_WIDE_WAVES), 1);
  return n;
}
static Wide wgrad_wide_auto(const ConvShape& cs) {
  const int Kout = cs.KH * cs.KW * cs.Cin;
  const int nt = cs.Cout / TileWide::BN;
  const int tiles = ceil_div(Kout, TileWide::BM) * nt;
  const int cap = ceil_div(cs.N * cs.OH * cs.OW, 4 * BK);
  if (nt == 1 && Kout > WGRAD_WIDE_1TILE_MAXKOUT) return Wide::NO;
  if (cap < WGRAD_WIDE_DB_SLOTS / tiles) return Wide::NO;
  return tiles >= WGRAD_WIDE_SB_MINTILES ? Wide::SB : Wide::DB;
}
static Wide wgrad_wide(const ConvShape& cs) {
  if (cs.Cout % TileWide::BN != 0 || wgrad_wide_mode() == 0) return Wide::NO;
  Wide pick = wgrad_wide_auto(cs);
  if (wgrad_wide_mode() == 1 && pick == Wide::NO) return Wide::NO;
  if (wgrad_wide_buf() != 0)
    pick = wgrad_wide_buf() == 2 ? Wide::SB : Wide::DB;
  else if (pick == Wide::NO)
    pick = Wide::DB;
  return pick;
}

static WgradRoute wgrad_route(DT dt, const void* x, const void* dy,
                              const ConvShape& cs) {
  const bool p2 = all_pow2(cs);
  if (p2 && vec_ok(dt, x, cs.Cin) && vec_ok(dt, dy, cs.Cout)) {
    if (dt != DT::BF16) return WgradRoute::VEC;
    const Wide wide = wgrad_wide(cs);
    if (wide == Wide::NO) return WgradRoute::TR;
    return wide == Wide::SB ? WgradRoute::TR_WIDE_SB : WgradRoute::TR_WIDE_DB;
  }
  return p2 ? WgradRoute::POW2 : WgradRoute::GENERIC;
}

int conv2d_wgrad_zsplits(DT dt, const void* x, const void* dy,
                         const ConvShape& cs) {
  const int M = cs.N * cs.OH * cs.OW;
  const int Kout = cs.KH * cs.KW * cs.Cin;
  const int cap = std::max(ceil_div(M, 4 * BK), 1);
  if (wgrad_splits_pin() > 0) return std::min(wgrad_splits_pin(), cap);
  const WgradRoute route = wgrad_route(dt, x, dy, cs);
  if (route == WgradRoute::TR_WIDE_DB || route == WgradRoute::TR_WIDE_SB) {
    const int base = ceil_div(Kout, TileWide::BM) * (cs.Cout / TileWide::BN);
    const int slots = (route == WgradRoute::TR_WIDE_DB ? WGRAD_WIDE_DB_SLOTS
                                                       : WGRAD_WIDE_SB_SLOTS) *
                      wgrad_wide_waves();
    return std::max(std::min(cap, slots / base), 1);
  }
  int base = ceil_div(Kout, BM) * ceil_div(cs.Cout, BN);
  int want = 2048;
  int z = base >= want ? 1 : std::min(cap, ceil_div(want, base));
  return std::max(z, 1);
}

const char* conv2d_wgrad_route(DT dt, const void* x, const void* dy,
                               const ConvShape& cs) {
  switch (wgrad_route(dt, x, dy, cs)) {
    case WgradRoute::TR_WIDE_DB: return "k_conv_wgrad_tr_wide<db>";
    case WgradRoute::TR_WIDE_SB: return "k_conv_wgrad_tr_wide<sb>";
    case WgradRoute::TR: return "k_conv_wgrad_tr";
    case WgradRoute::VEC: return "k_conv_wgrad_vec";
    case WgradRoute::POW2: return "k_conv_wgrad<pow2>";
    default: return "k_conv_wgrad";
  }
}

void conv2d_wgrad_launch(DT dt, const void* x, const void* dy, void* dw_out,
                         DT out_dt, float* ws, int z, const void* zero16,
                         const ConvShape& cs, bool bias, hipStream_t s) {
  int Kout = cs.KH * cs.KW * cs.Cin;
  const int bias_row = bias ? 1 : 0;
  bool direct = z == 1 && out_dt == DT::F32;
  float* target = direct ? (float*)dw_out : ws;
  dim3 grid(ceil_div(Kout, BM), ceil_div(cs.Cout, BN), z);
  const WgradRoute route = wgrad_route(dt, x, dy, cs);
  dispatch_dt(dt, [&](auto tag) {
    using T = typename decltype(tag)::type;
    auto X = (const T*)x;
    auto DY = (const T*)dy;
    auto Z = (const T*)zero16;
    if constexpr (sizeof(T) == 2) {
      if (route == WgradRoute::TR_WIDE_DB || route == WgradRoute::TR_WIDE_SB)
        return launch(route == WgradRoute::TR_WIDE_DB
                          ? k_conv_wgrad_tr_wide<true>
                          : k_conv_wgrad_tr_wide<false>,
                      dim3(ceil_div(Kout, TileWide::BM),
                           cs.Cout / TileWide::BN, z),
                      s, X, DY, target, Z, cs, bias_row);
      if (route == WgradRoute::TR)
        return launch(k_conv_wgrad_tr, grid, s, X, DY, target, Z, cs,
                      bias_row);
    } else {
      if (route == WgradRoute::VEC)
        return launch(k_conv_wgrad_vec<T>, grid, s, X, DY, target, Z, cs,
                      bias_row);
    }
    launch(route == WgradRoute::POW2 ? k_conv_wgrad<T, true>
                                     : k_conv_wgrad<T, false>,
           grid, s, X, DY, target, cs, bias_row);
  });
  if (!direct)
    splitk_reduce_launch(ws, dw_out, out_dt, z,
                         (int64_t)(Kout + bias_row) * cs.Cout, s,
                         (int64_t)Kout * cs.Cout);
}

}
```

tnn_amd/csrc/elementwise.hip:

```cpp

#include "common.h"
#include "kernels.h"

namespace tnn {

template <typename T, typename F>
__global__ void k_ewise1(const T* __restrict__ x, T* __restrict__ y,
                         int64_t n, F f) {
  int64_t i = (int64_t)blockIdx.x * blockDim.x + threadIdx.x;
  int64_t stride = (int64_t)gridDim.x * blockDim.x;
  for (; i < n; i += stride) y[i] = VecIO<T>::from_f32(f(VecIO<T>::to_f32(x[i])));
}

static inline int ew_blocks(int64_t n) {
  int64_t b = (n + 255) / 256;
  return (int)(b < 2048 ? b : 2048);
}

template <typename T>
__global__ void k_act_fwd(const T* x, T* y, int64_t n, int kind) {
  int64_t i = (int64_t)blockIdx.x * blockDim.x + threadIdx.x;
  int64_t stride = (int64_t)gridDim.x * blockDim.x;
  for (; i < n; i += stride)
    y[i] = VecIO<T>::from_f32(act_apply(VecIO<T>::to_f32(x[i]), kind));
// ... 105 lines not shown
    hipLaunchKernelGGL(k_act_bwd<bf16>, dim3(ew_blocks(n)), dim3(256), 0, s,
                       (const bf16*)dy, (const bf16*)x, (const bf16*)y,
                       (bf16*)dx, n, kind);
}

template <typename T>
__global__ void k_relu_bwd_mask(const T* dy, const T* y, T* dx, int64_t n) {
  int64_t i = (int64_t)blockIdx.x * blockDim.x + threadIdx.x;
  int64_t stride = (int64_t)gridDim.x * blockDim.x;
  for (; i < n; i += stride)
    dx[i] = VecIO<T>::to_f32(y[i]) > 0.0f ? dy[i] : VecIO<T>::from_f32(0.0f);
}

void relu_bwd_mask_launch(DT dt, const void* dy, const void* y, void* dx,
                          int64_t n, hipStream_t s) {
  if (dt == DT::F32)
    hipLaunchKernelGGL(k_relu_bwd_mask<float>, dim3(ew_blocks(n)), dim3(256), 0,
                       s, (const float*)dy, (const float*)y, (float*)dx, n);
  else
    hipLaunchKernelGGL(k_relu_bwd_mask<bf16>, dim3(ew_blocks(n)), dim3(256), 0,
                       s, (const bf16*)dy, (const bf16*)y, (bf16*)dx, n);
}

template <typename T>
__global__ void k_dropout_fwd(const T* x, T* y, uint8_t* mask, int64_t n,
                              float p, uint64_t seed,
                              const int64_t* __restrict__ ctr) {
  if (ctr) seed ^= (uint64_t)(*ctr) * 0x9E3779B97F4A7C15ull;
  const float scale = 1.0f / (1.0f - p);
  Philox rng(seed);
  int64_t i4 = (int64_t)blockIdx.x * blockDim.x + threadIdx.x;
  int64_t stride = (int64_t)gridDim.x * blockDim.x;
  for (; i4 * 4 < n; i4 += stride) {
    uint4 r = rng(i4);
    unsigned int rs[4] = {r.x, r.y, r.z, r.w};
#pragma unroll
    for (int j = 0; j < 4; ++j) {
      int64_t i = i4 * 4 + j;
      if (i < n) {
        bool keep = u32_to_uniform(rs[j]) > p;
        mask[i] = keep;
        y[i] = keep ? VecIO<T>::from_f32(VecIO<T>::to_f32(x[i]) * scale)
                    : VecIO<T>::from_f32(0.0f);
      }
    }
  }
}

template <typename T>
__global__ void k_dropout_bwd(const T* dy, const uint8_t* mask, T* dx,
                              int64_t n, float p) {
  const float scale = 1.0f / (1.0f - p);
  int64_t i = (int64_t)blockIdx.x * blockDim.x + threadIdx.x;
  int64_t stride = (int64_t)gridDim.x * blockDim.x;
  for (; i < n; i += stride)
    dx[i] = mask[i] ? VecIO<T>::from_f32(VecIO<T>::to_f32(dy[i]) * scale)
                    : VecIO<T>::from_f32(0.0f);
}

void dropout_fwd_launch(DT dt, const void* x, void* y, uint8_t* mask,
                        int64_t n, float p, uint64_t seed,
                        const int64_t* ctr, hipStream_t s) {
  int blocks = ew_blocks((n + 3) / 4);
  if (dt == DT::F32)
    hipLaunchKernelGGL(k_dropout_fwd<float>, dim3(blocks), dim3(256), 0, s,
                       (const float*)x, (float*)y, mask, n, p, seed, ctr);
  else
    hipLaunchKernelGGL(k_dropout_fwd<bf16>, dim3(blocks), dim3(256), 0, s,
                       (const bf16*)x, (bf16*)y, mask, n, p, seed, ctr);
}

void dropout_bwd_launch(DT dt, const void* dy, const uint8_t* mask, void* dx,
                        int64_t n, float p, hipStream_t s) {
  if (dt == DT::F32)
    hipLaunchKernelGGL(k_dropout_bwd<float>, dim3(ew_blocks(n)), dim3(256), 0,
                       s, (const float*)dy, mask, (float*)dx, n, p);
  else
    hipLaunchKernelGGL(k_dropout_bwd<bf16>, dim3(ew_blocks(n)), dim3(256), 0,
                       s, (const bf16*)dy, mask, (bf16*)dx, n, p);
}

template <int CPB>
__global__ void k_slab_fin(const float* __restrict__ ws,
                           float* __restrict__ out, int S, int C2) {
  constexpr int RPB = 256 / CPB;
  __shared__ float sh[256];
  const int cl = threadIdx.x % CPB;
  const int sl = threadIdx.x / CPB;
  const int c = blockIdx.x * CPB + cl;
  float a = 0.0f;
  if (c < C2)
    for (int s = sl; s < S; s += RPB) a += ws[(int64_t)s * C2 + c];
  sh[sl * CPB + cl] = a;
  __syncthreads();
  for (int h = RPB / 2; h > 0; h >>= 1) {
    if (sl < h) sh[sl * CPB + cl] += sh[(sl + h) * CPB + cl];
    __syncthreads();
  }
  if (sl == 0 && c < C2) out[c] = sh[cl];
}

void slab_fin_launch(const float* ws, float* out, int slices, int c2,
                     hipStream_t s) {
#define SLAB_CASE(CPB)                                                       \
  hipLaunchKernelGGL(k_slab_fin<CPB>, dim3((c2 + CPB - 1) / CPB), dim3(256), \
                     0, s, ws, out, slices, c2)
  if (c2 >= 128 * 32) SLAB_CASE(32);
  else if (c2 >= 128 * 16) SLAB_CASE(16);
  else if (c2 >= 128 * 8) SLAB_CASE(8);
  else if (c2 >= 128 * 4) SLAB_CASE(4);
  else if (c2 >= 128 * 2) SLAB_CASE(2);
  else SLAB_CASE(1);
#undef SLAB_CASE
}

template <typename T>
__global__ void k_colsum(const T* __restrict__ x, float* __restrict__ out,
                         int64_t rows, int cols) {
  const int col = blockIdx.x * 64 + (threadIdx.x & 63);
  const int rslice = blockIdx.y;
  const int nrs = gridDim.y;
  const int64_t r0 = rows * rslice / nrs, r1 = rows * (rslice + 1) / nrs;
  float acc = 0.0f;
  if (col < cols) {
    float a1 = 0.0f, a2 = 0.0f, a3 = 0.0f;
    int64_t r = r0 + (threadIdx.x >> 6);
    for (; r + 12 < r1; r += 16) {
      acc += VecIO<T>::to_f32(x[r * cols + col]);
      a1 += VecIO<T>::to_f32(x[(r + 4) * cols + col]);
      a2 += VecIO<T>::to_f32(x[(r + 8) * cols + col]);
      a3 += VecIO<T>::to_f32(x[(r + 12) * cols + col]);
    }
    for (; r < r1; r += 4) acc += VecIO<T>::to_f32(x[r * cols + col]);
    acc += (a1 + a2) + a3;
  }
  __shared__ float sh[4][64];
  sh[threadIdx.x >> 6][threadIdx.x & 63] = acc;
  __syncthreads();
  if (threadIdx.x < 64 && col < cols) {
    float v = sh[0][threadIdx.x] + sh[1][threadIdx.x] + sh[2][threadIdx.x] +
              sh[3][threadIdx.x];
    if (nrs == 1)
      out[col] = v;
    else
      atomicAdd(&out[col], v);
  }
}

template <typename T>
__global__ void k_colsum_vec(const T* __restrict__ x, float* __restrict__ out,
                             int64_t rows, int cols) {
  constexpr int V = 16 / sizeof(T);
  struct alignas(16) P { T e[16 / sizeof(T)]; };
  const int groups = cols / V;
  const int gpb = min(groups, 256);
  const int rows_per_iter = 256 / gpb;
  const int g = threadIdx.x % gpb + blockIdx.x * gpb;
  const int r_off = threadIdx.x / gpb;
  __shared__ float sh[256 * V];
  float s[V] = {};
  if (g < groups && r_off < rows_per_iter) {
    const int64_t r0 = rows * blockIdx.y / gridDim.y;
    const int64_t r1 = rows * (blockIdx.y + 1) / gridDim.y;
#pragma unroll 4
    for (int64_t r = r0 + r_off; r < r1; r += rows_per_iter) {
      P v = *(const P*)&x[r * cols + (int64_t)g * V];
#pragma unroll
      for (int j = 0; j < V; ++j) s[j] += VecIO<T>::to_f32(v.e[j]);
    }
  }
#pragma unroll
  for (int j = 0; j < V; ++j) sh[threadIdx.x * V + j] = s[j];
  __syncthreads();
  const int cpb_total = gpb * V;
  for (int cl = threadIdx.x; cl < cpb_total; cl += 256) {
    int gl = cl / V, j = cl % V;
    float t = 0.0f;
    for (int r = 0; r < rows_per_iter; ++r) t += sh[(r * gpb + gl) * V + j];
    int c = blockIdx.x * cpb_total + cl;
    if (c >= cols) break;
    if (gridDim.y == 1)
      out[c] = t;
    else
      out[(int64_t)blockIdx.y * cols + c] = t;
  }
}

int colsum_ws_slices(DT dt, const void* x, int64_t rows, int64_t cols) {
  int V = dt == DT::F32 ? 4 : 8;
// ... 61 lines not shown
```

tnn_amd/csrc/gemm.hip:

```cpp

#include "common.h"
#include "kernels.h"
#include "tile_gemm.h"

namespace tnn {

using namespace tile;


template <typename T>
struct Epilogue {
  const T* bias;
  const T* resid;
  int ldc;
  int act;
  DEV float at(float v, int col, int64_t idx) const {
    if (bias) v += VecIO<T>::to_f32(bias[col]);
    if (act != ACT_LINEAR) v = act_apply(v, act);
    if (resid) v += VecIO<T>::to_f32(resid[idx]);
    return v;
  }
  DEV float operator()(float v, int row, int col) const {
    return at(v, col, (int64_t)row * ldc + col);
  }
};

template <typename T, int ROWS>
DEV void stage_rows(T* dst, const T* __restrict__ src, int row0, int nrows,
                    int k0, int K) {
  constexpr int V = 16 / sizeof(T);
#pragma unroll
  for (int c = threadIdx.x; c < ROWS * (BK / V); c += THREADS) {
    int row = c / (BK / V);
    int kk = (c % (BK / V)) * V;
    int g = row0 + row;
    Pack16<T> v = {};
    if (g < nrows) v = load16_guarded(&src[(int64_t)g * K], k0 + kk, K);
    *(Pack16<T>*)&dst[lds_off<T>(row, kk)] = v;
  }
}

template <typename T, int ROWS>
DEV void glds_stage_rows(T* dst, const WaveCoord& wc,
                         const T* __restrict__ src,
                         const T* __restrict__ zero16, int row0, int nrows,
                         int K, int k0, int k_hi) {
  glds_stage<T, ROWS>(dst, wc, [&](int rl, int kk) -> const T* {
    int g = row0 + rl, gk = k0 + kk;
    if (g >= nrows || gk >= k_hi) return zero16;
    return &src[(int64_t)g * K + gk];
  });
}

template <typename T, int COLS>
DEV void stage_transposed(T* dst, const T* src, int ld, int k0,
                          int k_end, int c0) {
  constexpr int V = 16 / sizeof(T);
#pragma unroll 1
  for (int c = threadIdx.x; c < BK * (COLS / V); c += THREADS) {
    int kk = c / (COLS / V);
    int cc = (c % (COLS / V)) * V;
    int gk = k0 + kk;
    Pack16<T> v = {};
    if (gk < k_end) v = load16_guarded(&src[(int64_t)gk * ld], c0 + cc, ld);
#pragma unroll
    for (int j = 0; j < V; ++j)
      dst[lds_off<T>(cc + j, kk)] = v.e[j];
  }
}

template <typename T>
DEV void epilogue_store(const WaveCoord& wc, f32x4 acc[FM][FN], T* C, int m0,
                        int n0, int M, int N, const Epilogue<T>& ep) {
  epilogue_visit(wc, acc, m0, n0, [&](int row, int col, float v) {
    if (row < M && col < N)
      C[(int64_t)row * N + col] = VecIO<T>::from_f32(ep(v, row, col));
  });
}

DEV void slab_store(const WaveCoord& wc, f32x4 acc[FM][FN], float* ws,
                    int row0, int col0, int rows, int cols) {
  float* out = ws + (int64_t)blockIdx.z * rows * cols;
  epilogue_visit(wc, acc, row0, col0, [&](int row, int col, float v) {
// ... 960 lines not shown
                              const T* __restrict__ zero16, int M, int N,
                              int K) {
  constexpr int V = 16 / sizeof(T);
  constexpr int RA = BK * (BM / V) / THREADS;
  constexpr int RB = BK * (BN / V) / THREADS;
  __shared__ alignas(16) T As[BM * BK];
  __shared__ alignas(16) T Bs[BN * BK];
  const int r0 = blockIdx.x * BM;
  const int n0 = blockIdx.y * BN;
  const int m_begin = (int)((int64_t)M * blockIdx.z / gridDim.z);
  const int m_end = (int)((int64_t)M * (blockIdx.z + 1) / gridDim.z);
  const WaveCoord wc;
  f32x4 acc[FM][FN] = {};
  using VecT = Pack16<T>;

  for (int k0 = m_begin; k0 < m_end; k0 += BK) {
    constexpr bool TR = sizeof(T) == 2;
    const int a_rr = TR ? (threadIdx.x & (BM / V - 1)) * V : 0;
    const int a_mm0 = TR ? (threadIdx.x / (BM / V)) * 4 : 0;
    const T* asrc[RA];
#pragma unroll
    for (int it = 0; it < RA; ++it) {
      int mm, rr;
      if constexpr (TR) {
        mm = a_mm0 + it;
        rr = a_rr;
      } else {
        int c = threadIdx.x + it * THREADS;
        mm = c / (BM / V);
        rr = (c % (BM / V)) * V;
      }
      int gm = k0 + mm, gr = r0 + rr;
      asrc[it] = (gm < m_end && gr < K) ? &A[(int64_t)gm * K + gr] : zero16;
    }
    const T* bsrc[RB];
#pragma unroll
    for (int it = 0; it < RB; ++it) {
      int c = threadIdx.x + it * THREADS;
      int mm = c / (BN / V);
      int nn = (c % (BN / V)) * V;
      int gm = k0 + mm, gn = n0 + nn;
      bsrc[it] = (gm < m_end && gn < N) ? &B[(int64_t)gm * N + gn] : zero16;
    }
    VecT va[RA], vb[RB];
#pragma unroll
    for (int it = 0; it < RA; ++it) va[it] = *(const VecT*)asrc[it];
#pragma unroll
    for (int it = 0; it < RB; ++it) vb[it] = *(const VecT*)bsrc[it];
    if constexpr (TR) {
#pragma unroll
      for (int j = 0; j < V; ++j) {
        struct alignas(8) H4 { T e[4]; } h;
#pragma unroll
        for (int q = 0; q < 4; ++q) h.e[q] = va[q].e[j];
        *(H4*)&As[lds_off<T>(a_rr + j, a_mm0)] = h;
      }
    } else {
#pragma unroll
      for (int it = 0; it < RA; ++it) {
        int c = threadIdx.x + it * THREADS;
        int mm = c / (BM / V);
        int rr = (c % (BM / V)) * V;
#pragma unroll
        for (int j = 0; j < V; ++j) As[lds_off<T>(rr + j, mm)] = va[it].e[j];
      }
    }
#pragma unroll
    for (int it = 0; it < RB; ++it) {
      int c = threadIdx.x + it * THREADS;
      int mm = c / (BN / V);
      int nn = (c % (BN / V)) * V;
#pragma unroll
      for (int j = 0; j < V; ++j) Bs[lds_off<T>(nn + j, mm)] = vb[it].e[j];
    }
    __syncthreads();
    mfma_compute_tile(As, Bs, wc, acc);
    __syncthreads();
  }

  slab_store(wc, acc, C, r0, n0, K, N);
}

template <typename OUT>
__global__ void k_splitk_reduce(const float* __restrict__ ws,
                                OUT* __restrict__ out, int z, int64_t n) {
  int64_t i = (int64_t)blockIdx.x * blockDim.x + threadIdx.x;
  int64_t stride = (int64_t)gridDim.x * blockDim.x;
  for (; i < n; i += stride) {
    float acc = 0.0f;
    for (int s = 0; s < z; ++s) acc += ws[(int64_t)s * n + i];
    out[i] = VecIO<OUT>::from_f32(acc);
  }
}

template <typename OUT>
__global__ void k_splitk_reduce4(const float4* __restrict__ ws,
                                 OUT* __restrict__ out, int z, int64_t n4) {
  int64_t i = (int64_t)blockIdx.x * blockDim.x + threadIdx.x;
  int64_t stride = (int64_t)gridDim.x * blockDim.x;
  for (; i < n4; i += stride) {
    float4 a0{0, 0, 0, 0}, a1{0, 0, 0, 0}, a2{0, 0, 0, 0}, a3{0, 0, 0, 0};
    int s = 0;
    for (; s + 4 <= z; s += 4) {
      float4 v0 = ws[(int64_t)s * n4 + i];
      float4 v1 = ws[(int64_t)(s + 1) * n4 + i];
      float4 v2 = ws[(int64_t)(s + 2) * n4 + i];
      float4 v3 = ws[(int64_t)(s + 3) * n4 + i];
      a0.x += v0.x; a0.y += v0.y; a0.z += v0.z; a0.w += v0.w;
      a1.x += v1.x; a1.y += v1.y; a1.z += v1.z; a1.w += v1.w;
      a2.x += v2.x; a2.y += v2.y; a2.z += v2.z; a2.w += v2.w;
      a3.x += v3.x; a3.y += v3.y; a3.z += v3.z; a3.w += v3.w;
    }
    for (; s < z; ++s) {
      float4 v = ws[(int64_t)s * n4 + i];
      a0.x += v.x; a0.y += v.y; a0.z += v.z; a0.w += v.w;
    }
    float r[4];
    r[0] = (a0.x + a1.x) + (a2.x + a3.x);
    r[1] = (a0.y + a1.y) + (a2.y + a3.y);
    r[2] = (a0.z + a1.z) + (a2.z + a3.z);
    r[3] = (a0.w + a1.w) + (a2.w + a3.w);
    struct alignas(4 * sizeof(OUT)) O4 { OUT e[4]; } o;
#pragma unroll
    for (int j = 0; j < 4; ++j) o.e[j] = VecIO<OUT>::from_f32(r[j]);
    ((O4*)out)[i] = o;
  }
}

template <typename OUT, int CPB>
__global__ void k_splitk_fold(const float4* __restrict__ ws,
                              OUT* __restrict__ out, int z, int64_t n4) {
  constexpr int RPB = 256 / CPB;
  __shared__ float4 sh[256];
  const int cl = threadIdx.x % CPB;
  const int r = threadIdx.x / CPB;
  const int64_t c = (int64_t)blockIdx.x * CPB + cl;
  float4 a{0.0f, 0.0f, 0.0f, 0.0f};
  if (c < n4)
    for (int sl = r; sl < z; sl += RPB) {
      float4 v = ws[(int64_t)sl * n4 + c];
      a.x += v.x; a.y += v.y; a.z += v.z; a.w += v.w;
    }
  sh[r * CPB + cl] = a;
  __syncthreads();
  for (int h = RPB / 2; h > 0; h >>= 1) {
    if (r < h) {
      float4 o = sh[(r + h) * CPB + cl];
      float4 m = sh[r * CPB + cl];
      m.x += o.x; m.y += o.y; m.z += o.z; m.w += o.w;
      sh[r * CPB + cl] = m;
    }
    __syncthreads();
  }
  if (r == 0 && c < n4) {
    float4 m = sh[cl];
    struct alignas(4 * sizeof(OUT)) O4 { OUT e[4]; } o;
    o.e[0] = VecIO<OUT>::from_f32(m.x);
    o.e[1] = VecIO<OUT>::from_f32(m.y);
    o.e[2] = VecIO<OUT>::from_f32(m.z);
    o.e[3] = VecIO<OUT>::from_f32(m.w);
    ((O4*)out)[c] = o;
  }
}

template <typename OUT>
static void splitk_fold_launch(const float4* ws, OUT* out, int z, int64_t n4,
                               hipStream_t s, int64_t n4_shape) {
#define FOLD_CASE(CPB)                                                    \
  hipLaunchKernelGGL((k_splitk_fold<OUT, CPB>),                           \
                     dim3((unsigned)((n4 + CPB - 1) / CPB)), dim3(256), 0, \
                     s, ws, out, z, n4)
  if (n4_shape >= 128 * 32) FOLD_CASE(32);
  else if (n4_shape >= 128 * 16) FOLD_CASE(16);
  else if (n4_shape >= 128 * 8) FOLD_CASE(8);
  else if (n4_shape >= 128 * 4) FOLD_CASE(4);
  else if (n4_shape >= 128 * 2) FOLD_CASE(2);
  else FOLD_CASE(1);
#undef FOLD_CASE
}

void splitk_reduce_launch(const float* ws, void* out, DT out_dt, int z,
                          int64_t n, hipStream_t s, int64_t n_shape) {
  if (n_shape <= 0) n_shape = n;
  dispatch_dt(out_dt, [&](auto tag) {
    using OUT = typename decltype(tag)::type;
    if ((n & 3) == 0 && (n_shape & 3) == 0 && n_shape < 4 * 32768 && z >= 8) {
      splitk_fold_launch((const float4*)ws, (OUT*)out, z, n >> 2, s,
                         n_shape >> 2);
    } else if ((n & 3) == 0) {
      int64_t n4 = n >> 2;
      int blocks = (int)std::min<int64_t>((n4 + 255) / 256, (int64_t)2048);
      hipLaunchKernelGGL(k_splitk_reduce4<OUT>, dim3(blocks), dim3(256), 0, s,
                         (const float4*)ws, (OUT*)out, z, n4);
    } else {
      int blocks = (int)std::min<int64_t>((n + 255) / 256, (int64_t)2048);
      hipLaunchKernelGGL(k_splitk_reduce<OUT>, dim3(blocks), dim3(256), 0, s,
                         ws, (OUT*)out, z, n);
    }
  });
}


void gemm_launch(DT dt, const void* a, const void* b, const void* bias,
                 void* c, const void* zero16, const void* resid, int M, int N,
                 int K, bool trans_b, int act_kind, hipStream_t s) {
  dispatch_dt(dt, [&](auto tag) {
    using T = typename decltype(tag)::type;
    const T* A = (const T*)a;
    const T* B = (const T*)b;
    if (M == 1 && trans_b) {
      hipLaunchKernelGGL(k_gemv_nt<T>, dim3(ceil_div(N, 4)), dim3(256), 0, s,
                         A, B, (const T*)bias, (const T*)resid, (T*)c, N, K,
                         act_kind);
      return;
    }
    dim3 grid(ceil_div(M, BM), ceil_div(N, BN));
    const bool g = K % vec_elems(dt) == 0 && ptr_aligned16(a) &&
                   (!trans_b || ptr_aligned16(b));
    auto launch = [&](auto kern) {
      hipLaunchKernelGGL(kern, grid, dim3(THREADS), 0, s, A, B,
                         (const T*)bias, (T*)c, (const T*)zero16,
                         (const T*)resid, M, N, K, act_kind);
    };
    if (trans_b && g && K <= 3072)
      launch(k_gemm_nt_db<T>);
    else if (trans_b)
      launch(g ? k_gemm<T, true, true> : k_gemm<T, true, false>);
    else
      launch(g ? k_gemm<T, false, true> : k_gemm<T, false, false>);
  });
}

int gemv_nn_ksplits(int N, int K) {
  int ncb = ceil_div(N, 256);
  int ks = std::max(1, 512 / ncb);
  ks = std::min(ks, std::max(1, K / 16));
  return ks;
}

void gemv_nn_launch(DT dt, const void* x, const void* b, const void* bias,
                    void* y, float* ws, int ks, int N, int K, int act_kind,
                    hipStream_t s) {
  dim3 pg(ceil_div(N, 256), ks);
  dim3 fg(ceil_div(N, 256));
  dispatch_dt(dt, [&](auto tag) {
    using T = typename decltype(tag)::type;
    hipLaunchKernelGGL(k_gemv_nn_part<T>, pg, dim3(256), 0, s, (const T*)x,
                       (const T*)b, ws, N, K);
    hipLaunchKernelGGL(k_gemv_nn_fin<T>, fg, dim3(256), 0, s, ws,
                       (const T*)bias, (T*)y, N, ks, act_kind);
  });
}

int gemm_tn_zsplits(int M, int N, int K) {
  int base = ceil_div(K, BM) * ceil_div(N, BN);
  int want = 2048;
  int z = base >= want ? 1 : std::min(ceil_div(M, BK), ceil_div(want, base));
  return std::max(z, 1);
}

void gemm_tn_launch(DT dt, const void* a, const void* b, void* c_out,
                    DT out_dt, float* ws, int z, const void* zero16, int M,
                    int N, int K, hipStream_t s) {
  dim3 grid(ceil_div(K, BM), ceil_div(N, BN), z);
  bool direct = z == 1 && out_dt == DT::F32;
  float* target = direct ? (float*)c_out : ws;
  const int V = vec_elems(dt);
  const bool vec = K % V == 0 && N % V == 0 && ptr_aligned16(a) &&
                   ptr_aligned16(b);
  dispatch_dt(dt, [&](auto tag) {
    using T = typename decltype(tag)::type;
    if (vec)
      hipLaunchKernelGGL(k_gemm_tn_vec<T>, grid, dim3(THREADS), 0, s,
                         (const T*)a, (const T*)b, target, (const T*)zero16,
                         M, N, K);
    else
      hipLaunchKernelGGL(k_gemm_tn<T>, grid, dim3(THREADS), 0, s, (const T*)a,
                         (const T*)b, target, M, N, K);
  });
  if (!direct)
// ... 41 lines not shown
```

tnn_amd/csrc/kernels.h:

```cpp
#pragma once

#include <hip/hip_runtime.h>
#ifdef __HIPCC__
#include <hip/hip_bf16.h>
#endif
#include <algorithm>
#include <cstdint>

namespace tnn {

enum class DT { F32, BF16 };

inline bool ptr_aligned16(const void* p) { return ((uintptr_t)p & 15) == 0; }

inline int vec_elems(DT dt) { return dt == DT::F32 ? 4 : 8; }

#ifdef __HIPCC__
template <typename T> struct TypeTag { using type = T; };
template <typename F>
inline void dispatch_dt(DT dt, F&& f) {
  if (dt == DT::F32) f(TypeTag<float>{});
  else f(TypeTag<__hip_bfloat16>{});
}
#endif

void act_fwd_launch(DT dt, const void* x, void* y, int64_t n, int kind,
                    hipStream_t s);
void act_bwd_launch(DT dt, const void* dy, const void* x, const void* y,
                    void* dx, int64_t n, int kind, hipStream_t s);
void add_act_fwd_launch(DT dt, const void* a, const void* b, void* y,
                        int64_t n, int kind, hipStream_t s);
void add_act_bwd_launch(DT dt, const void* dy, const void* y, void* g,
                        int64_t n, int kind, hipStream_t s);
void relu_bwd_mask_launch(DT dt, const void* dy, const void* y, void* dx,
                          int64_t n, hipStream_t s);
void dropout_fwd_launch(DT dt, const void* x, void* y, uint8_t* mask,
                        int64_t n, float p, uint64_t seed,
                        const int64_t* ctr, hipStream_t s);
void dropout_bwd_launch(DT dt, const void* dy, const uint8_t* mask, void* dx,
                        int64_t n, float p, hipStream_t s);
int colsum_ws_slices(DT dt, const void* x, int64_t rows, int64_t cols);
void colsum_launch(DT dt, const void* x, void* out_f32, float* ws,
                   int rslices, int64_t rows, int64_t cols, hipStream_t s);
void slab_fin_launch(const float* ws, float* out, int slices, int c2,
                     hipStream_t s);
void cast_f32_launch(DT dt_out, const float* x, void* y, int64_t n,
                     hipStream_t s);

void gemm_launch(DT dt, const void* a, const void* b, const void* bias,
                 void* c, const void* zero16, const void* resid, int M, int N,
                 int K, bool trans_b, int act_kind, hipStream_t s);
int gemv_nn_ksplits(int N, int K);
int gemv_nn1_nsplit(int N, int K);
void gemv_nn1_launch(DT dt, const void* x, const void* b, const void* bias,
                     const void* res, void* y, float* part, int nsplit,
                     const float* ln_g, const float* ln_b, float ln_eps, int N,
                     int K, int act_kind, hipStream_t s);
constexpr int GEMV1_MAX_K = 8192;
constexpr int SKINNY_MAX_M = 16;
int gemm_skinny_nsplit(DT dt, int M, int N, int K);
void gemm_skinny_launch(DT dt, const void* x, const void* b, const void* bias,
                        const void* res, void* y, float* part, int nsplit,
                        const float* ln_g, const float* ln_b, float ln_eps,
                        int M, int N, int K, int act_kind, hipStream_t s);
void gemv_nn_launch(DT dt, const void* x, const void* b, const void* bias,
                    void* y, float* ws, int ks, int N, int K, int act_kind,
                    hipStream_t s);
int gemm_nt_zsplits(DT dt, int M, int N, int K);
int gemm_nt_fsplits(DT dt, int M, int N, int K);
int gemm_nt32_zsplits(int M, int N, int K);
void gemm_nt32_launch(const void* a, const void* b, float* ws,
                      const void* bias, const void* resid, void* c, int z,
                      const void* zero16, int M, int N, int K, int act_kind,
                      hipStream_t s);
void gemm_nt_zf_launch(DT dt, const void* a, const void* b, float* ws,
                       const void* bias, const void* resid, void* c, int z,
                       const void* zero16, int M, int N, int K, int act_kind,
                       hipStream_t s);
void gemm_nt_z_launch(DT dt, const void* a, const void* b, float* ws,
                      void* c_out, DT out_dt, int z, const void* zero16,
                      int M, int N, int K, hipStream_t s);
int gemm_tn_zsplits(int M, int N, int K);
void gemm_tn_launch(DT dt, const void* a, const void* b, void* c_out,
                    DT out_dt, float* ws, int z, const void* zero16, int M,
                    int N, int K, hipStream_t s);
void splitk_reduce_launch(const float* ws, void* out, DT out_dt, int z,
                          int64_t n, hipStream_t s, int64_t n_shape = 0);
void mfma_selftest_launch(const void* a_bf16, const void* b_bf16, float* d,
                          hipStream_t s);
void mfma_selftest_f32_launch(const float* a, const float* b, float* d,
                              hipStream_t s);

struct IDiv {
  int d = 1;
  int lg = 0;
  int sh = 0;
  unsigned long long magic = 0;
  void set(int dd) {
    d = dd;
    lg = (dd & (dd - 1)) == 0 ? __builtin_ctz(dd) : -1;
    magic = 0;
    sh = 0;
    if (lg < 0 && dd > 1 && dd < 65536) {
      sh = dd < 1024 ? 36 : 42;
      magic = ((1ull << sh) + dd - 1) / dd;
    }
  }
};

struct ConvShape {
  int N, H, W, Cin, Cout, KH, KW, SH, SW, PH, PW, OH, OW;
  IDiv d_ohow, d_ow, d_cin, d_hw, d_w, d_cout;
  int mkw16;
  void init_fdiv() {
    d_ohow.set(OH * OW);
    d_ow.set(OW);
    d_cin.set(Cin);
    d_hw.set(H * W);
    d_w.set(W);
    d_cout.set(Cout);
    mkw16 = 65536 / KW + 1;
  }
};
bool conv2d_fwd_wants_db(DT dt, const void* x, const ConvShape& cs);
void transpose_w_fwd_launch(DT dt, const void* w, void* w_t2, int KHW, int Cin,
                            int Cout, hipStream_t s);
void conv2d_fwd_launch(DT dt, const void* x, const void* w, const void* w_t2,
                       const void* bias, void* y, const void* zero16,
                       float* stats, const ConvShape& cs, bool relu,
                       hipStream_t s);
bool conv2d_dgrad_wants_db(DT dt, const void* dy, const ConvShape& cs);
const char* conv2d_fwd_route(DT dt, const void* x, const ConvShape& cs,
                             bool stats);
const char* conv2d_dgrad_route(DT dt, const void* dy, const ConvShape& cs);
void transpose_w_dgrad_launch(DT dt, const void* w, void* w_t2d, int KHW,
                              int Cin, int Cout, hipStream_t s);
void conv2d_dgrad_launch(DT dt, const void* dy, const void* w_t,
                         const void* w_t2d, void* dx, const void* zero16,
                         const ConvShape& cs, hipStream_t s);
const char* conv2d_wgrad_route(DT dt, const void* x, const void* dy,
                               const ConvShape& cs);
int conv2d_wgrad_zsplits(DT dt, const void* x, const void* dy,
                         const ConvShape& cs);
void conv2d_wgrad_launch(DT dt, const void* x, const void* dy, void* dw_out,
                         DT out_dt, float* ws, int z, const void* zero16,
                         const ConvShape& cs, bool bias, hipStream_t s);
void transpose_w_launch(DT dt, const void* w, void* w_t, int KH, int KW,
                        int Cin, int Cout, hipStream_t s);

int64_t bn_stats_ws_floats(DT dt, const void* x, int64_t rows, int cols);
void bn_stats_launch(DT dt, const void* x, float* mean, float* invstd,
                     float* rmean, float* rvar, float momentum, float* ws,
                     int64_t rows, int cols, float eps, hipStream_t s);
void bn_finalize_launch(const float* sum, const float* sumsq, float* mean,
                        float* invstd, float* rmean, float* rvar,
                        float momentum, int64_t rows, int cols, float eps,
                        hipStream_t s);
void bn_apply_launch(DT dt, const void* x, const float* mean,
                     const float* invstd, const float* gamma, const float* beta,
                     void* y, int64_t rows, int cols, bool relu, hipStream_t s);
void bn_apply_drop_launch(DT dt, const void* x, const float* mean,
                          const float* invstd, const float* gamma,
                          const float* beta, void* y, int64_t rows, int cols,
                          float p, uint64_t seed, const int64_t* ctr,
                          hipStream_t s);
void bn_infer_launch(DT dt, const void* x, const float* rmean,
                     const float* rvar, const float* gamma, const float* beta,
                     void* y, int64_t rows, int cols, float eps, bool relu,
                     hipStream_t s);
int64_t bn_bwd_ws_floats(DT dt, const void* x, const void* dy, int64_t rows,
                         int cols);
void bn_bwd_reduce_launch(DT dt, const void* x, const void* dy, const void* y_relu,
                          const float* mean, const float* invstd, float* sum_dy,
                          float* sum_dy_xhat, float* ws, int64_t rows, int cols,
                          float dy_scale, hipStream_t s);
void bn_bwd_apply_launch(DT dt, const void* x, const void* dy, const void* y_relu,
                         const float* mean, const float* invstd,
                         const float* gamma, const float* sum_dy,
                         const float* sum_dy_xhat, void* dx, const void* resid,
                         int64_t rows, int cols, float dy_scale,
                         hipStream_t s);

struct PoolShape {
  int N, H, W, C, KH, KW, SH, SW, PH, PW, OH, OW;
};
void maxpool_fwd_launch(DT dt, const void* x, void* y, int32_t* idx,
                        const PoolShape& ps, hipStream_t s);
void maxpool_bwd_launch(DT dt, const void* dy, const int32_t* idx, float* dx_f32,
                        const PoolShape& ps, hipStream_t s);
void avgpool_fwd_launch(DT dt, const void* x, void* y, const PoolShape& ps,
                        hipStream_t s);
void avgpool_bwd_launch(DT dt, const void* dy, void* dx, const PoolShape& ps,
                        hipStream_t s);

void ce_fwd_launch(DT dt, const void* logits, const int64_t* targets,
                   float* loss, float* lse, int64_t rows, int cols,
                   hipStream_t s);
void ce_bwd_launch(DT dt, const void* logits, const int64_t* targets,
                   const float* lse, const float* dloss, void* dlogits,
                   int64_t rows, int cols, hipStream_t s);
void ptloss_fwd_launch(DT dt, const void* pred, const void* tgt, float* out,
                       int64_t n, int kind, float delta, hipStream_t s);
void ptloss_bwd_launch(DT dt, const void* pred, const void* tgt,
                       const float* dloss, void* dpred, int64_t n, int kind,
                       float delta, hipStream_t s);

void gn_fwd_launch(DT dt, const void* x, const float* gamma, const float* beta,
                   void* y, float* mean, float* invstd, int64_t N, int64_t HW,
                   int C, int G, float eps, hipStream_t s);
void gn_bwd_launch(DT dt, const void* x, const void* dy, const float* mean,
                   const float* invstd, const float* gamma, float* s1,
                   float* s2, void* dx, float* dgamma, float* dbeta, int64_t N,
                   int64_t HW, int C, int G, hipStream_t s);

void ln_fwd_launch(DT dt, const void* x, const float* gamma, const float* beta,
                   void* y, float* mean, float* invstd, int64_t rows, int cols,
                   float eps, hipStream_t s);
int64_t ln_bwd_ws_floats(DT dt, const void* x, const void* dy, int64_t rows,
                         int cols);
void ln_bwd_launch(DT dt, const void* x, const void* dy, const float* gamma,
                   const float* mean, const float* invstd, void* dx,
                   const void* resid, float* dgamma2, float* ws, int64_t rows,
                   int cols, hipStream_t s);

void embedding_fwd_launch(DT dt, const int64_t* ids, const void* table,
                          void* y, int64_t n_ids, int dim, hipStream_t s);
void embedding_bwd_launch(DT dt, const int64_t* ids, const void* dy,
                          float* dtable_f32, int64_t n_ids, int dim,
                          hipStream_t s);

void attn_fwd_launch(const void* q, const void* k, const void* v, void* o,
                     float* lse, const void* zero16, int B, int H, int S,
                     int D, const int64_t* i_str, const int64_t* o_str,
                     bool causal, float scale, hipStream_t s);
void attn_bwd_launch(const void* q, const void* k, const void* v,
                     const void* o, const void* dout, const float* lse,
                     float* di, float* dq_ws, void* dq, void* dk, void* dv,
                     const void* zero16, int B, int H, int S, int D,
                     const int64_t* i_str, const int64_t* o_str,
                     const int64_t* do_str, const int64_t* w_str, bool causal,
                     float scale, hipStream_t s);
void attn_ext_launch(const void* q, const void* k, const void* v, void* o,
                     const int64_t* pos, const int64_t* n_new,
                     const void* zero16, int B, int H, int T, int cap, int D,
                     const int64_t* q_str, const int64_t* o_str, float scale,
                     hipStream_t s);

void bmm_launch(DT dt, const void* a, const void* b, void* c,
                const void* zero16, int batch, int M, int N, int K, int lda,
                int ldb, int ldc, int64_t sa, int64_t sb, int64_t sc, bool ta,
                bool tb, hipStream_t s);

void smax_fwd_launch(DT dt, const void* x, void* y, int64_t rows, int cols,
                     int mrows, int qoff, float scale, bool causal,
                     hipStream_t s);
void smax_bwd_launch(DT dt, const void* p, const void* dy, void* dx,
                     int64_t rows, int cols, float scale, hipStream_t s);

// ... 47 lines not shown
```

tnn_amd/ops/functional.py:

```python

from __future__ import annotations

from typing import Optional, Tuple

import torch
import torch.nn.functional as F

from .. import _C


ACT_KINDS = {
    "linear": 0,
    "relu": 1,
    "gelu": 2,
    "sigmoid": 3,
    "tanh": 4,
    "elu": 5,
    "leaky_relu": 6,
    "silu": 7,
}


def _nhwc_to_nchw(x: torch.Tensor) -> torch.Tensor:
    return x.permute(0, 3, 1, 2)


def _nchw_to_nhwc(x: torch.Tensor) -> torch.Tensor:
    return x.permute(0, 2, 3, 1).contiguous()


def _use_hip(*tensors: torch.Tensor) -> bool:
    return any(t is not None and t.is_cuda for t in tensors)


_graph_ctr: Optional[torch.Tensor] = None


def set_graph_seed_ctr(t: Optional[torch.Tensor]):
    global _graph_ctr
    _graph_ctr = t


def _draw_seed() -> int:
    if _graph_ctr is not None:
        import random
        return random.getrandbits(62)
    return int(torch.randint(0, 2 ** 62, (1,)).item())




class _Conv2dNHWC(torch.autograd.Function):
    @staticmethod
    def forward(ctx, x, w, bias, stride, padding, fuse_relu, want_stats=False):
        ext = _C.ext()
        Ci = x.shape[-1]
        V = 8 if x.dtype == torch.bfloat16 else 4
        ctx.cin = Ci
        if Ci % V != 0 and Ci < V:
            x = F.pad(x, (0, V - Ci))
            w = F.pad(w, (0, 0, 0, V - Ci))
        ctx.want_stats = want_stats
        if want_stats:
            y, stats = ext.conv2d_fwd_stats(x, w, bias, stride[0], stride[1],
                                            padding[0], padding[1])
        else:
            y = ext.conv2d_fwd(x, w, bias, stride[0], stride[1], padding[0],
                               padding[1], fuse_relu)
        ctx.save_for_backward(x, w, y if fuse_relu else None)
        ctx.stride, ctx.padding, ctx.fuse_relu = stride, padding, fuse_relu
        ctx.has_bias = bias is not None
        if want_stats:
            ctx.mark_non_differentiable(stats)
            return y, stats
        return y

    @staticmethod
    def backward(ctx, dy, *unused_stats_grad):
        x, w, y = ctx.saved_tensors
        ext = _C.ext()
        dy = dy.contiguous()
        if ctx.fuse_relu:
            dy = ext.relu_bwd_mask(dy, y)
        dx = dw = db = None
        if ctx.needs_input_grad[0]:
            dx = ext.conv2d_dgrad(dy, w, x.shape[1], x.shape[2],
                                  ctx.stride[0], ctx.stride[1], ctx.padding[0], ctx.padding[1])
            if x.shape[-1] != ctx.cin:
                dx = dx[..., :ctx.cin].contiguous()
        want_db = ctx.has_bias and ctx.needs_input_grad[2]
        if ctx.needs_input_grad[1]:
            args = (x, dy, w.shape[0], w.shape[1], ctx.stride[0],
                    ctx.stride[1], ctx.padding[0], ctx.padding[1],
                    w.dtype == x.dtype)
            if want_db:
                dw, db = ext.conv2d_wgrad_bias(*args)
                db = db.to(dy.dtype)
            else:
                dw = ext.conv2d_wgrad(*args)
            if x.shape[-1] != ctx.cin:
                dw = dw[:, :, :ctx.cin].contiguous()
            dw = dw.to(w.dtype)
        elif want_db:
            db = ext.colsum(dy.reshape(-1, dy.shape[-1]))
        return dx, dw, db, None, None, None, None


def conv2d_nhwc(
    x: torch.Tensor,
    w: torch.Tensor,
    bias: Optional[torch.Tensor] = None,
    stride: Tuple[int, int] = (1, 1),
    padding: Tuple[int, int] = (0, 0),
    fuse_relu: bool = False,
    want_stats: bool = False,
):
    if _use_hip(x):
        if want_stats:
            y, stats = _Conv2dNHWC.apply(
                x.contiguous(), w.contiguous(),
                None if bias is None else bias.contiguous(), stride, padding,
                False, True)
            return y, (stats if stats.numel() else None)
        return _Conv2dNHWC.apply(x.contiguous(), w.contiguous(),
                                 None if bias is None else bias.contiguous(),
                                 stride, padding, fuse_relu)
    wn = w.permute(3, 2, 0, 1)
    y = F.conv2d(_nhwc_to_nchw(x), wn, bias, stride=stride, padding=padding)
    if want_stats:
        return _nchw_to_nhwc(y), None
    y = _nchw_to_nhwc(y)
    if fuse_relu:
        y = F.relu(y)
    return y




class _BatchNormAct(torch.autograd.Function):
    @staticmethod
    def forward(ctx, x, gamma, beta, running_mean, running_var, momentum,
                eps, relu, dropout_p=0.0, seed=0, precomp=None, ctr=None):
        ext = _C.ext()
        y, mean, invstd = ext.bn_fwd_train(x, gamma, beta, running_mean,
                                           running_var, momentum, eps, relu,
                                           dropout_p, seed, precomp, ctr)
        save_y = y if (relu or dropout_p > 0.0) else None
        ctx.save_for_backward(x, gamma, mean, invstd, save_y)
        ctx.relu = relu or dropout_p > 0.0
        ctx.dy_scale = 1.0 / (1.0 - dropout_p) if dropout_p > 0.0 else 1.0
        ctx.mark_non_differentiable(mean, invstd)
        return y, mean, invstd

    @staticmethod
    def backward(ctx, dy, _dmean, _dinvstd):
        x, gamma, mean, invstd, y = ctx.saved_tensors
        ext = _C.ext()
        dx, dgamma, dbeta = ext.bn_bwd(x, dy.contiguous(), gamma, mean, invstd,
                                       y if ctx.relu else None, ctx.dy_scale)
        return (dx, dgamma, dbeta, None, None, None, None, None, None, None,
                None, None)


class _BatchNormActRes(torch.autograd.Function):

    @staticmethod
    def forward(ctx, x, gamma, beta, running_mean, running_var, momentum,
                eps, relu, dropout_p, seed, precomp, ctr):
        ext = _C.ext()
        y, mean, invstd = ext.bn_fwd_train(x, gamma, beta, running_mean,
                                           running_var, momentum, eps, relu,
                                           dropout_p, seed, precomp, ctr)
        save_y = y if (relu or dropout_p > 0.0) else None
        ctx.save_for_backward(x, gamma, mean, invstd, save_y)
        ctx.relu = relu or dropout_p > 0.0
        ctx.dy_scale = 1.0 / (1.0 - dropout_p) if dropout_p > 0.0 else 1.0
        ctx.mark_non_differentiable(mean, invstd)
        ctx.set_materialize_grads(False)
        return y, mean, invstd, x.view_as(x)

    @staticmethod
    def backward(ctx, dy, _dm, _di, dres):
        x, gamma, mean, invstd, y = ctx.saved_tensors
        ext = _C.ext()
        if dy is None:
            return (dres, None, None, None, None, None, None, None, None,
                    None, None, None)
        if dres is not None:
            dres = dres.contiguous()
        dx, dgamma, dbeta = ext.bn_bwd(x, dy.contiguous(), gamma, mean,
                                       invstd, y if ctx.relu else None,
                                       ctx.dy_scale, resid=dres)
        return (dx, dgamma, dbeta, None, None, None, None, None, None, None,
                None, None)


def batch_norm_act(
    x: torch.Tensor,
    gamma: torch.Tensor,
    beta: torch.Tensor,
    running_mean: torch.Tensor,
    running_var: torch.Tensor,
    training: bool,
    momentum: float = 0.1,
    eps: float = 1e-5,
    relu: bool = False,
    dropout_p: float = 0.0,
    precomputed: Optional[torch.Tensor] = None,
    passthrough: bool = False,
):
    C = x.shape[-1]
    n = x.numel() // C
    if _use_hip(x):
        if training:
            seed = _draw_seed() if dropout_p > 0.0 else 0
            if passthrough:
                y, _, _, xr = _BatchNormActRes.apply(
                    x.contiguous(), gamma, beta, running_mean, running_var,
                    momentum, eps, relu, dropout_p, seed, precomputed,
                    _graph_ctr)
                return y, xr
            y, _, _ = _BatchNormAct.apply(x.contiguous(), gamma, beta,
                                          running_mean, running_var, momentum,
                                          eps, relu, dropout_p, seed,
                                          precomputed, _graph_ctr)
            return y
        ext = _C.ext()
        return ext.bn_fwd_infer(x.contiguous(), gamma, beta, running_mean, running_var,
                                eps, relu)
    xf = x.reshape(-1, C).float()
    if training:
        mean = xf.mean(0)
        var = xf.var(0, unbiased=False)
        with torch.no_grad():
            running_mean.mul_(1 - momentum).add_(mean.detach(), alpha=momentum)
            running_var.mul_(1 - momentum).add_(var.detach() * (n / max(n - 1, 1)),
                                                alpha=momentum)
    else:
        mean, var = running_mean, running_var
    xhat = (x.float() - mean) / torch.sqrt(var + eps)
    y = xhat * gamma + beta
    if relu:
        y = F.relu(y)
    if dropout_p > 0.0 and training:
        y = F.dropout(y, dropout_p, training=True)
    y = y.to(x.dtype)
    return (y, x) if passthrough else y




class _Linear(torch.autograd.Function):

    @staticmethod
    def forward(ctx, x, w, bias, act, residual=None):
        ext = _C.ext()
        y = ext.gemm(x, w, bias, ACT_KINDS[act], residual)
        ctx.save_for_backward(x, w, y if act != "linear" else None)
        ctx.act = act
        ctx.has_bias = bias is not None
        ctx.has_res = residual is not None
        return y

    @staticmethod
    def backward(ctx, dy):
        x, w, y = ctx.saved_tensors
        ext = _C.ext()
        dy = dy.contiguous()
        dres = dy if ctx.has_res else None
        if ctx.act == "relu":
            assert not ctx.has_res, \
                "fused residual requires act='linear' (relu mask would include it)"
            dy = ext.relu_bwd_mask(dy, y)
        elif ctx.act != "linear":
            raise NotImplementedError(f"fused act bwd for {ctx.act}")
# ... 704 lines not shown
```

tnn_amd/utils/graphstep.py:

```python

from __future__ import annotations


import torch


class GraphedInference:
    def __init__(self, model: torch.nn.Module, example_input: torch.Tensor,
                 warmup: int = 3):
        assert example_input.is_cuda, "graph capture needs GPU tensors"
        self.model = model
        model.eval()
        self.static_in = example_input.clone()
        stream = torch.cuda.Stream()
        stream.wait_stream(torch.cuda.current_stream())
        with torch.cuda.stream(stream):
            with torch.no_grad():
                for _ in range(warmup):
                    out = model(self.static_in)
        torch.cuda.current_stream().wait_stream(stream)
        self.graph = torch.cuda.CUDAGraph()
        with torch.no_grad():
            with torch.cuda.graph(self.graph):
                self.static_out = model(self.static_in)

    @torch.no_grad()
    def __call__(self, x: torch.Tensor) -> torch.Tensor:
        self.static_in.copy_(x)
        self.graph.replay()
        return self.static_out


class GraphedTrainStep:

    def __init__(self, model, criterion, optimizer, example_x, example_y,
                 warmup: int = 3):
        from ..ops.functional import set_graph_seed_ctr
        assert example_x.is_cuda
        self.model, self.criterion, self.optimizer = model, criterion, optimizer
        self.static_x = example_x.clone()
        self.static_y = example_y.clone()
        dev = example_x.device
        self.step_ctr = torch.zeros(1, dtype=torch.int64, device=dev)
        model.train()
        optimizer._step_dev = self.step_ctr
        self.lr_dev = torch.full((1,), float(optimizer.lr),
                                 dtype=torch.float32, device=dev)
        self._lr_written = optimizer.lr
        optimizer._lr_dev = self.lr_dev
        groups = {}
        for prm in optimizer.params:
            groups.setdefault(prm.dtype, []).append(prm)
        self._grad_slabs = []
        for dt, ps in groups.items():
            slab = torch.zeros(sum(pp.numel() for pp in ps), dtype=dt,
                               device=dev)
            off = 0
            for pp in ps:
                pp.grad = slab[off:off + pp.numel()].view_as(pp)
                off += pp.numel()
            self._grad_slabs.append(slab)
        set_graph_seed_ctr(self.step_ctr)
        try:
            stream = torch.cuda.Stream()
            stream.wait_stream(torch.cuda.current_stream())
            with torch.cuda.stream(stream):
                for _ in range(warmup):
                    self._step_body()
            torch.cuda.current_stream().wait_stream(stream)
            self.graph = torch.cuda.CUDAGraph()
            with torch.cuda.graph(self.graph):
                self.static_loss = self._step_body()
        finally:
            set_graph_seed_ctr(None)

    def _step_body(self):
        self.step_ctr.add_(1)
        for slab in self._grad_slabs:
            slab.zero_()
        out = self.model(self.static_x)
        loss = self.criterion(out, self.static_y)
        loss.backward()
        self.optimizer.step()
        return loss

    def __call__(self, x=None, y=None) -> torch.Tensor:
        if x is not None:
            self.static_x.copy_(x)
        if y is not None:
            self.static_y.copy_(y)
        if self.optimizer.lr != self._lr_written:
            self.lr_dev.fill_(float(self.optimizer.lr))
            self._lr_written = self.optimizer.lr
        self.graph.replay()
        return self.static_loss

    def sync_step_count(self):
        self.optimizer.step_count = int(self.step_ctr.item())
```

Measured before the change: 43980 img/s.

## Write BN and conv weight gradients directly into grad slabs and fold stats partials

Adds gradient sinks: conv wgrad and BN backward write or accumulate their parameter gradients straight into the pre-allocated grad slab, so the separate autograd accumulation copies go away. The graphed train step now zeros only the slab ranges that sinks do not write. Conv forward stats are emitted as per-tile partials, and a new fold kernel reduces them inside the BN finalize step instead of using atomics into a zeroed buffer. In exchange there is more bookkeeping, and the code relies on every step writing the same set of parameters, which is checked with an assertion.

Result: faster. 45870 img/s, median of 6 (+4.3%).

```diff
diff --git a/tnn_amd/csrc/batchnorm.hip b/tnn_amd/csrc/batchnorm.hip
--- a/tnn_amd/csrc/batchnorm.hip
+++ b/tnn_amd/csrc/batchnorm.hip
@@ -168,6 +168,22 @@
   }
 }
 
+DEV void bn_finalize_channel(int c, float sum, float sumsq, float shift,
+                             float* mean, float* invstd, float* rmean,
+                             float* rvar, float momentum, int64_t rows,
+                             float eps) {
+  float d = sum / rows;
+  float var = fmaxf(sumsq / rows - d * d, 0.0f);
+  float m = shift + d;
+  mean[c] = m;
+  invstd[c] = rsqrtf(var + eps);
+  if (rmean) {
+    float unbiased = var * ((float)rows / (float)(rows > 1 ? rows - 1 : 1));
+    rmean[c] = rmean[c] * (1.0f - momentum) + m * momentum;
+    rvar[c] = rvar[c] * (1.0f - momentum) + unbiased * momentum;
+  }
+}
+
 template <typename T>
 __global__ void k_bn_finalize(float* mean, float* invstd, const float* sum,
                               const float* sumsq, const T* shift, float* rmean,
@@ -175,16 +191,42 @@
                               int cols, float eps) {
   int c = blockIdx.x * blockDim.x + threadIdx.x;
   if (c >= cols) return;
-  float d = sum[c] / rows;
-  float var = fmaxf(sumsq[c] / rows - d * d, 0.0f);
-  float m = shift ? VecIO<T>::to_f32(shift[c]) + d : d;
-  mean[c] = m;
-  invstd[c] = rsqrtf(var + eps);
-  if (rmean) {
-    float unbiased = var * ((float)rows / (float)(rows > 1 ? rows - 1 : 1));
-    rmean[c] = rmean[c] * (1.0f - momentum) + m * momentum;
-    rvar[c] = rvar[c] * (1.0f - momentum) + unbiased * momentum;
-  }
+  if (shift)
+    bn_finalize_channel(c, sum[c], sumsq[c], VecIO<T>::to_f32(shift[c]), mean,
+                        invstd, rmean, rvar, momentum, rows, eps);
+  else
+    bn_finalize_channel(c, sum[c], sumsq[c], 0.0f, mean, invstd, rmean, rvar,
+                        momentum, rows, eps);
+}
+
+template <int CPB>
+__global__ void k_bn_finalize_fold(const float* __restrict__ part, int S,
+                                   float* mean, float* invstd, float* rmean,
+                                   float* rvar, float momentum, int64_t rows,
+                                   int C, float eps) {
+  constexpr int RPB = 256 / CPB;
+  __shared__ float sh[2][256];
+  const int cl = threadIdx.x % CPB;
+  const int sl = threadIdx.x / CPB;
+  const int c = blockIdx.x * CPB + cl;
+  float a = 0.0f, b = 0.0f;
+  if (c < C) {
+    for (int s = sl; s < S; s += RPB) a += part[(int64_t)s * 2 * C + c];
+    for (int s = sl; s < S; s += RPB) b += part[(int64_t)s * 2 * C + C + c];
+  }
+  sh[0][sl * CPB + cl] = a;
+  sh[1][sl * CPB + cl] = b;
+  __syncthreads();
+  for (int h = RPB / 2; h > 0; h >>= 1) {
+    if (sl < h) {
+      sh[0][sl * CPB + cl] += sh[0][(sl + h) * CPB + cl];
+      sh[1][sl * CPB + cl] += sh[1][(sl + h) * CPB + cl];
+    }
+    __syncthreads();
+  }
+  if (sl == 0 && c < C)
+    bn_finalize_channel(c, sh[0][cl], sh[1][cl], 0.0f, mean, invstd, rmean,
+                        rvar, momentum, rows, eps);
 }
 
 template <typename T>
@@ -499,6 +541,24 @@
                      eps);
 }
 
+void bn_finalize_fold_launch(const float* partials, int slices, float* mean,
+                             float* invstd, float* rmean, float* rvar,
+                             float momentum, int64_t rows, int cols, float eps,
+                             hipStream_t s) {
+  const int c2 = 2 * cols;
+#define FOLD_CASE(CPB)                                                       \
+  hipLaunchKernelGGL(k_bn_finalize_fold<CPB>, dim3((cols + CPB - 1) / CPB), \
+                     dim3(256), 0, s, partials, slices, mean, invstd, rmean, \
+                     rvar, momentum, rows, cols, eps)
+  if (c2 >= 128 * 32) FOLD_CASE(32);
+  else if (c2 >= 128 * 16) FOLD_CASE(16);
+  else if (c2 >= 128 * 8) FOLD_CASE(8);
+  else if (c2 >= 128 * 4) FOLD_CASE(4);
+  else if (c2 >= 128 * 2) FOLD_CASE(2);
+  else FOLD_CASE(1);
+#undef FOLD_CASE
+}
+
 void bn_apply_launch(DT dt, const void* x, const float* mean,
                      const float* invstd, const float* gamma, const float* beta,
                      void* y, int64_t rows, int cols, bool relu,
@@ -592,7 +652,9 @@
                           const void* y_relu, const float* mean,
                           const float* invstd, float* sum_dy,
                           float* sum_dy_xhat, float* ws, int64_t rows,
-                          int cols, float dy_scale, hipStream_t s) {
+                          int cols, float dy_scale, hipStream_t s,
+                          float* dgamma_out, float* dbeta_out,
+                          bool accumulate) {
   if (ws) {
     dim3 g = dt == DT::F32 ? bn_reduce_grid_vec<float>(rows, cols)
                            : bn_reduce_grid_vec<bf16>(rows, cols);
@@ -605,7 +667,8 @@
       hipLaunchKernelGGL(k_bn_bwd_reduce_vec<bf16>, g, dim3(256), 0, s,
                          (const bf16*)x, (const bf16*)dy, (const bf16*)y_relu,
                          mean, invstd, ws, nullptr, rows, cols, dy_scale);
-    slab_fin_launch(ws, sum_dy, (int)g.y, 2 * cols, s);
+    slab_fin_launch(ws, sum_dy, (int)g.y, 2 * cols, s, dbeta_out, dgamma_out,
+                    accumulate);
     return;
   }
   if (dt == DT::F32)
diff --git a/tnn_amd/csrc/bindings.cpp b/tnn_amd/csrc/bindings.cpp
--- a/tnn_amd/csrc/bindings.cpp
+++ b/tnn_amd/csrc/bindings.cpp
@@ -500,7 +500,8 @@
                            cs.KH * cs.KW, cs.Cin, cs.Cout, cur_stream());
   }
   if (want_stats)
-    stats = db ? at::zeros({2, (int64_t)cs.Cout},
+    stats = db ? at::empty({(int64_t)conv2d_fwd_stats_rows(cs), 2,
+                            (int64_t)cs.Cout},
                            x.options().dtype(at::kFloat))
                : at::empty({0}, x.options().dtype(at::kFloat));
   conv2d_fwd_launch(dt_of(x), x.data_ptr(), w.data_ptr(),
@@ -523,6 +524,21 @@
                                          const c10::optional<at::Tensor>& bias,
                                          int64_t sh, int64_t sw, int64_t ph,
                                          int64_t pw) {
+  auto out = conv2d_fwd_impl(x, w, bias, sh, sw, ph, pw, false, true);
+  if (out[1].numel()) {
+    auto stats = at::empty({2, out[1].size(2)}, out[1].options());
+    slab_fin_launch(out[1].data_ptr<float>(), stats.data_ptr<float>(),
+                    (int)out[1].size(0), (int)(2 * out[1].size(2)),
+                    cur_stream());
+    out[1] = stats;
+  }
+  return out;
+}
+
+std::vector<at::Tensor> conv2d_fwd_partials(
+    const at::Tensor& x, const at::Tensor& w,
+    const c10::optional<at::Tensor>& bias, int64_t sh, int64_t sw, int64_t ph,
+    int64_t pw) {
   return conv2d_fwd_impl(x, w, bias, sh, sw, ph, pw, false, true);
 }
 
@@ -612,6 +628,68 @@
   const int64_t kout = out.size(0) - 1;
   return {out.narrow(0, 0, kout).view({KH, KW, x.size(3), dy.size(3)}),
           out.select(0, kout)};
+}
+
+static void check_grad_dst(const char* fn, const char* name,
+                           const at::Tensor& t, const at::Tensor& like,
+                           at::ScalarType st, at::IntArrayRef shape) {
+  TORCH_CHECK(t.is_cuda() && t.device() == like.device(), fn, ": ", name,
+              " must be a GPU tensor on ", like.device());
+  TORCH_CHECK(t.scalar_type() == st, fn, ": ", name, " must be ", st, ", got ",
+              t.scalar_type());
+  TORCH_CHECK(t.sizes() == shape, fn, ": ", name, " must have shape ", shape,
+              ", got ", t.sizes());
+  TORCH_CHECK(t.is_contiguous(), fn, ": ", name, " must be contiguous");
+}
+
+bool splitk_can_split(int64_t n, int64_t n0, int64_t addr0, int64_t addr1,
+                      bool bf16_out) {
+  return splitk_reduce_can_split(n, n0, (const void*)(uintptr_t)addr0,
+                                 (const void*)(uintptr_t)addr1,
+                                 bf16_out ? DT::BF16 : DT::F32);
+}
+
+void conv2d_wgrad_into(const at::Tensor& x, const at::Tensor& dy, int64_t KH,
+                       int64_t KW, int64_t sh, int64_t sw, int64_t ph,
+                       int64_t pw, at::Tensor dw_out,
+                       const c10::optional<at::Tensor>& db_out,
+                       bool accumulate) {
+  const char* fn = "conv2d_wgrad_into";
+  auto cs = conv_wgrad_shape(fn, x, dy, KH, KW, sh, sw, ph, pw);
+  const auto st = dw_out.scalar_type();
+  TORCH_CHECK(st == x.scalar_type() || st == at::kFloat, fn,
+              ": dw_out must be ", x.scalar_type(), " or Float, got ", st);
+  check_grad_dst(fn, "dw_out", dw_out, x, st,
+                 {KH, KW, (int64_t)cs.Cin, (int64_t)cs.Cout});
+  const bool bias = db_out.has_value();
+  if (bias) check_grad_dst(fn, "db_out", *db_out, x, st, {(int64_t)cs.Cout});
+  const DT out_dt = st == at::kFloat ? DT::F32 : dt_of(x);
+  const int64_t kout = KH * KW * cs.Cin;
+  const int64_t rows = kout + (bias ? 1 : 0);
+  const int z = conv2d_wgrad_zsplits(dt_of(x), x.data_ptr(), dy.data_ptr(), cs);
+  auto ws = at::empty({(int64_t)z * rows * cs.Cout},
+                      x.options().dtype(at::kFloat));
+  void* dbp = bias ? db_out->data_ptr() : nullptr;
+  if (splitk_reduce_can_split(rows * cs.Cout, kout * cs.Cout,
+                              dw_out.data_ptr(), bias ? dbp : dw_out.data_ptr(),
+                              out_dt)) {
+    WgradSink sink{dbp, accumulate};
+    conv2d_wgrad_launch(dt_of(x), x.data_ptr(), dy.data_ptr(),
+                        dw_out.data_ptr(), out_dt, ws.data_ptr<float>(), z,
+                        zero_page(x), cs, bias, cur_stream(), &sink);
+    return;
+  }
+  auto tmp = at::empty({rows, (int64_t)cs.Cout}, ws.options());
+  WgradSink one{nullptr, false};
+  conv2d_wgrad_launch(dt_of(x), x.data_ptr(), dy.data_ptr(), tmp.data_ptr(),
+                      DT::F32, ws.data_ptr<float>(), z, zero_page(x), cs, bias,
+                      cur_stream(), &one);
+  auto put = [&](at::Tensor dst, const at::Tensor& src) {
+    dst.copy_(accumulate ? dst.to(at::kFloat).add_(src.view(dst.sizes()))
+                         : src.view(dst.sizes()));
+  };
+  put(dw_out, tmp.narrow(0, 0, kout));
+  if (bias) put(*db_out, tmp.select(0, kout));
 }
 
 std::vector<at::Tensor> bn_fwd_train(const at::Tensor& x,
@@ -634,11 +712,25 @@
   float* rm = rmean.has_value() ? rmean->data_ptr<float>() : nullptr;
   float* rv = rvar.has_value() ? rvar->data_ptr<float>() : nullptr;
   if (precomp.has_value()) {
-    TORCH_CHECK(precomp->numel() == 2 * C, "bad precomputed stats");
+    TORCH_CHECK(precomp->is_cuda() && precomp->is_contiguous() &&
+                    precomp->scalar_type() == at::kFloat,
+                "bn_fwd_train: precomp must be a contiguous fp32 GPU tensor");
+    const bool partials = precomp->dim() == 3;
+    TORCH_CHECK(partials ? precomp->size(0) >= 1 && precomp->size(1) == 2 &&
+                               precomp->size(2) == C
+                         : precomp->numel() == 2 * C,
+                "bad precomputed stats: ", precomp->sizes(), " for C = ", C);
     const float* ps = precomp->data_ptr<float>();
-    bn_finalize_launch(ps, ps + C, mean.data_ptr<float>(),
-                       invstd.data_ptr<float>(), rm, rv, (float)momentum,
-                       rows, C, (float)eps, cur_stream());
+    if (partials)
+      bn_finalize_fold_launch(ps, (int)precomp->size(0),
+                              mean.data_ptr<float>(),
+                              invstd.data_ptr<float>(), rm, rv,
+                              (float)momentum, rows, C, (float)eps,
+                              cur_stream());
+    else
+      bn_finalize_launch(ps, ps + C, mean.data_ptr<float>(),
+                         invstd.data_ptr<float>(), rm, rv, (float)momentum,
+                         rows, C, (float)eps, cur_stream());
   } else {
     const int64_t wsn = bn_stats_ws_floats(dt_of(x), x.data_ptr(), rows, C);
     at::Tensor ws;
@@ -686,7 +778,12 @@
                                const c10::optional<at::Tensor>& y_relu,
                                double dy_scale,
                                const c10::optional<at::Tensor>& resid =
-                                   c10::nullopt) {
+                                   c10::nullopt,
+                               const c10::optional<at::Tensor>& dgamma_out =
+                                   c10::nullopt,
+                               const c10::optional<at::Tensor>& dbeta_out =
+                                   c10::nullopt,
+                               bool accumulate = false) {
   CHECK_IN(x);
   CHECK_IN(dy);
   const void* resp = nullptr;
@@ -704,6 +801,17 @@
                   : at::zeros({2, C}, x.options().dtype(at::kFloat));
   auto sum_dy = sums[0];
   auto sum_dy_xhat = sums[1];
+  float *dgp = nullptr, *dbp = nullptr;
+  TORCH_CHECK(dgamma_out.has_value() == dbeta_out.has_value(),
+              "bn_bwd: dgamma_out and dbeta_out go together");
+  if (dgamma_out.has_value()) {
+    TORCH_CHECK(wsn, "bn_bwd: no gradient sink on the scalar path "
+                     "(ask bn_bwd_takes_sink first)");
+    check_grad_dst("bn_bwd", "dgamma_out", *dgamma_out, x, at::kFloat, {C});
+    check_grad_dst("bn_bwd", "dbeta_out", *dbeta_out, x, at::kFloat, {C});
+    dgp = dgamma_out->data_ptr<float>();
+    dbp = dbeta_out->data_ptr<float>();
+  }
   at::Tensor ws;
   float* wp = nullptr;
   if (wsn) {
@@ -715,13 +823,22 @@
   bn_bwd_reduce_launch(dt_of(x), x.data_ptr(), dy.data_ptr(), yr,
                        mean.data_ptr<float>(), invstd.data_ptr<float>(),
                        sum_dy.data_ptr<float>(), sum_dy_xhat.data_ptr<float>(),
-                       wp, rows, C, (float)dy_scale, cur_stream());
+                       wp, rows, C, (float)dy_scale, cur_stream(), dgp, dbp,
+                       accumulate);
   bn_bwd_apply_launch(dt_of(x), x.data_ptr(), dy.data_ptr(), yr,
                       mean.data_ptr<float>(), invstd.data_ptr<float>(),
                       gamma.data_ptr<float>(), sum_dy.data_ptr<float>(),
                       sum_dy_xhat.data_ptr<float>(), dx.data_ptr(), resp,
                       rows, C, (float)dy_scale, cur_stream());
   return {dx, sum_dy_xhat, sum_dy};
+}
+
+bool bn_bwd_takes_sink(const at::Tensor& x, const at::Tensor& dy) {
+  CHECK_IN(x);
+  CHECK_IN(dy);
+  const int C = x.size(-1);
+  return bn_bwd_ws_floats(dt_of(x), x.data_ptr(), dy.data_ptr(),
+                          x.numel() / C, C) != 0;
 }
 
 static PoolShape pool_shape(const at::Tensor& x, int KH, int KW, int SH, int SW,
@@ -1465,12 +1582,19 @@
   m.def("mfma_selftest_f32", &tnn::mfma_selftest_f32);
   m.def("conv2d_fwd", &tnn::conv2d_fwd);
   m.def("conv2d_fwd_stats", &tnn::conv2d_fwd_stats);
+  m.def("conv2d_fwd_partials", &tnn::conv2d_fwd_partials);
   m.def("conv2d_dgrad", &tnn::conv2d_dgrad);
   m.def("conv2d_fwd_route", &tnn::conv2d_fwd_route_name);
   m.def("conv2d_dgrad_route", &tnn::conv2d_dgrad_route_name);
   m.def("conv2d_wgrad_route", &tnn::conv2d_wgrad_route_name);
   m.def("conv2d_wgrad", &tnn::conv2d_wgrad);
   m.def("conv2d_wgrad_bias", &tnn::conv2d_wgrad_bias);
+  m.def("conv2d_wgrad_into", &tnn::conv2d_wgrad_into, py::arg("x"),
+        py::arg("dy"), py::arg("KH"), py::arg("KW"), py::arg("sh"),
+        py::arg("sw"), py::arg("ph"), py::arg("pw"), py::arg("dw_out"),
+        py::arg("db_out") = py::none(), py::arg("accumulate") = false);
+  m.def("bn_bwd_takes_sink", &tnn::bn_bwd_takes_sink);
+  m.def("splitk_can_split", &tnn::splitk_can_split);
   m.def("bn_fwd_train", &tnn::bn_fwd_train, py::arg("x"), py::arg("gamma"),
         py::arg("beta"), py::arg("rmean"), py::arg("rvar"),
         py::arg("momentum"), py::arg("eps"), py::arg("relu"),
@@ -1480,7 +1604,8 @@
   m.def("bn_bwd", &tnn::bn_bwd, py::arg("x"), py::arg("dy"),
         py::arg("gamma"), py::arg("mean"), py::arg("invstd"),
         py::arg("y_relu"), py::arg("dy_scale"),
-        py::arg("resid") = py::none());
+        py::arg("resid") = py::none(), py::arg("dgamma_out") = py::none(),
+        py::arg("dbeta_out") = py::none(), py::arg("accumulate") = false);
   m.def("maxpool_fwd", &tnn::maxpool_fwd);
   m.def("maxpool_bwd", &tnn::maxpool_bwd);
   m.def("avgpool_fwd", &tnn::avgpool_fwd);
diff --git a/tnn_amd/csrc/conv2d.hip b/tnn_amd/csrc/conv2d.hip
--- a/tnn_amd/csrc/conv2d.hip
+++ b/tnn_amd/csrc/conv2d.hip
@@ -195,16 +195,17 @@
 
 template <typename T, typename S>
 DEV void conv_fwd_stats(const WaveCoordT<S>& wc, f32x4 acc[S::FM][S::FN],
-                        const T* bias_p, float* stats, const ConvShape& cs,
-                        int m0, int n0, int M) {
+                        const T* bias_p, float* partials, const ConvShape& cs,
+                        int tm, int m0, int n0, int M) {
   constexpr int FM = S::FM, FN = S::FN;
-  float* ssum = stats;
-  float* ssumsq = stats + cs.Cout;
+  __shared__ float red[2][S::WAVES_M][S::BN];
+  const int wm = wc.wid / S::WAVES_N;
   const int cr = (wc.lane >> 4) * 4;
   const int cc = wc.lane & 15;
 #pragma unroll
   for (int fn = 0; fn < FN; ++fn) {
-    int col = n0 + wc.wcol0 + fn * 16 + cc;
+    const int lcol = wc.wcol0 + fn * 16 + cc;
+    int col = n0 + lcol;
     float bias = 0.0f;
     if (col < cs.Cout) {
       if (bias_p) bias = VecIO<T>::to_f32(bias_p[col]);
@@ -225,10 +226,20 @@
     ss += __shfl_xor(ss, 16, 64);
     s += __shfl_xor(s, 32, 64);
     ss += __shfl_xor(ss, 32, 64);
-    if (wc.lane < 16 && col < cs.Cout) {
-      atomicAdd(&ssum[col], s);
-      atomicAdd(&ssumsq[col], ss);
-    }
+    if (wc.lane < 16) {
+      red[0][wm][lcol] = s;
+      red[1][wm][lcol] = ss;
+    }
+  }
+  __syncthreads();
+  for (int i = threadIdx.x; i < 2 * S::BN; i += THREADS) {
+    const int which = i / S::BN, lcol = i % S::BN;
+    const int col = n0 + lcol;
+    if (col >= cs.Cout) continue;
+    float a = red[which][0][lcol];
+#pragma unroll
+    for (int w = 1; w < S::WAVES_M; ++w) a += red[which][w][lcol];
+    partials[((int64_t)tm * 2 + which) * cs.Cout + col] = a;
   }
 }
 
@@ -438,7 +449,8 @@
   }
 
   conv_fwd_store(wc, acc, bias, Y, cs, act_kind, m0, n0, M);
-  if constexpr (STATS) conv_fwd_stats(wc, acc, bias, stats, cs, m0, n0, M);
+  if constexpr (STATS)
+    conv_fwd_stats(wc, acc, bias, stats, cs, tm_, m0, n0, M);
 }
 
 template <typename T, bool STATS = false>
@@ -1067,6 +1079,11 @@
   return buf;
 }
 
+int conv2d_fwd_stats_rows(const ConvShape& cs) {
+  static_assert(TileWide::BM == BM, "one m-tile height for the partials");
+  return ceil_div(cs.N * cs.OH * cs.OW, BM);
+}
+
 enum class Wide { NO, DB, SB };
 constexpr int WIDE_MIN_TILES = 512;
 constexpr int WIDE_FWD_DB_MINK = 2048;
@@ -1077,10 +1094,10 @@
   if (wide_buf() != 0) single = wide_buf() == 2;
   return single ? Wide::SB : Wide::DB;
 }
-static Wide fwd_wide(DT dt, bool have_wt2, const ConvShape& cs, bool stats) {
+static Wide fwd_wide(DT dt, bool have_wt2, const ConvShape& cs) {
   const int nt = cs.Cout / TileWide::BN;
   const int K = cs.KH * cs.KW * cs.Cin;
-  const bool take = nt == 1 ? !stats : K >= WIDE_FWD_DB_MINK;
+  const bool take = nt == 1 || K >= WIDE_FWD_DB_MINK;
   return wide_pick(
       have_wt2 && dt == DT::BF16 && cs.Cout % TileWide::BN == 0,
       ceil_div(cs.N * cs.OH * cs.OW, TileWide::BM) * nt, take, nt == 1);
@@ -1144,7 +1161,7 @@
 static FwdRoute fwd_route(DT dt, const void* x, bool have_wt2,
                           const ConvShape& cs, bool stats) {
   if (have_wt2) {
-    const Wide wide = fwd_wide(dt, true, cs, stats);
+    const Wide wide = fwd_wide(dt, true, cs);
     if (wide != Wide::NO)
       return wide == Wide::SB ? FwdRoute::SB_WIDE : FwdRoute::DB_WIDE;
     const bool long_k =
@@ -1398,10 +1415,11 @@
 
 void conv2d_wgrad_launch(DT dt, const void* x, const void* dy, void* dw_out,
                          DT out_dt, float* ws, int z, const void* zero16,
-                         const ConvShape& cs, bool bias, hipStream_t s) {
+                         const ConvShape& cs, bool bias, hipStream_t s,
+                         const WgradSink* sink) {
   int Kout = cs.KH * cs.KW * cs.Cin;
   const int bias_row = bias ? 1 : 0;
-  bool direct = z == 1 && out_dt == DT::F32;
+  bool direct = z == 1 && out_dt == DT::F32 && !sink;
   float* target = direct ? (float*)dw_out : ws;
   dim3 grid(ceil_div(Kout, BM), ceil_div(cs.Cout, BN), z);
   const WgradRoute route = wgrad_route(dt, x, dy, cs);
@@ -1433,7 +1451,9 @@
   if (!direct)
     splitk_reduce_launch(ws, dw_out, out_dt, z,
                          (int64_t)(Kout + bias_row) * cs.Cout, s,
-                         (int64_t)Kout * cs.Cout);
-}
-
-}
+                         (int64_t)Kout * cs.Cout,
+                         sink && bias ? sink->db_out : nullptr,
+                         (int64_t)Kout * cs.Cout, sink && sink->accumulate);
+}
+
+}
diff --git a/tnn_amd/csrc/elementwise.hip b/tnn_amd/csrc/elementwise.hip
--- a/tnn_amd/csrc/elementwise.hip
+++ b/tnn_amd/csrc/elementwise.hip
@@ -211,7 +211,9 @@
 
 template <int CPB>
 __global__ void k_slab_fin(const float* __restrict__ ws,
-                           float* __restrict__ out, int S, int C2) {
+                           float* __restrict__ out, int S, int C2,
+                           float* __restrict__ d0, float* __restrict__ d1,
+                           int acc) {
   constexpr int RPB = 256 / CPB;
   __shared__ float sh[256];
   const int cl = threadIdx.x % CPB;
@@ -226,14 +228,22 @@
     if (sl < h) sh[sl * CPB + cl] += sh[(sl + h) * CPB + cl];
     __syncthreads();
   }
-  if (sl == 0 && c < C2) out[c] = sh[cl];
+  if (sl == 0 && c < C2) {
+    const float v = sh[cl];
+    out[c] = v;
+    if (d0) {
+      const int C = C2 >> 1;
+      float* d = c < C ? d0 + c : d1 + (c - C);
+      *d = acc ? *d + v : v;
+    }
+  }
 }
 
 void slab_fin_launch(const float* ws, float* out, int slices, int c2,
-                     hipStream_t s) {
+                     hipStream_t s, float* d0, float* d1, bool accumulate) {
 #define SLAB_CASE(CPB)                                                       \
   hipLaunchKernelGGL(k_slab_fin<CPB>, dim3((c2 + CPB - 1) / CPB), dim3(256), \
-                     0, s, ws, out, slices, c2)
+                     0, s, ws, out, slices, c2, d0, d1, accumulate ? 1 : 0)
   if (c2 >= 128 * 32) SLAB_CASE(32);
   else if (c2 >= 128 * 16) SLAB_CASE(16);
   else if (c2 >= 128 * 8) SLAB_CASE(8);
diff --git a/tnn_amd/csrc/gemm.hip b/tnn_amd/csrc/gemm.hip
--- a/tnn_amd/csrc/gemm.hip
+++ b/tnn_amd/csrc/gemm.hip
@@ -1,4 +1,5 @@
 
+#include <stdexcept>
 #include "common.h"
 #include "kernels.h"
 #include "tile_gemm.h"
@@ -1125,20 +1126,56 @@
 }
 
 template <typename OUT>
-__global__ void k_splitk_reduce(const float* __restrict__ ws,
-                                OUT* __restrict__ out, int z, int64_t n) {
+struct SplitDst {
+  OUT* out0;
+  OUT* out1;
+  int64_t n0;
+  int acc;
+  __device__ OUT* at(int64_t i) const {
+    return i < n0 ? out0 + i : out1 + (i - n0);
+  }
+  __device__ OUT* at4(int64_t i4) const {
+    return i4 < n0 ? out0 + 4 * i4 : out1 + 4 * (i4 - n0);
+  }
+};
+
+template <typename OUT>
+__device__ inline void split_store4(const SplitDst<OUT>& d, int64_t i4,
+                                    float r0, float r1, float r2, float r3) {
+  struct alignas(4 * sizeof(OUT)) O4 { OUT e[4]; };
+  O4* p = (O4*)d.at4(i4);
+  if (d.acc) {
+    O4 g = *p;
+    r0 += VecIO<OUT>::to_f32(g.e[0]);
+    r1 += VecIO<OUT>::to_f32(g.e[1]);
+    r2 += VecIO<OUT>::to_f32(g.e[2]);
+    r3 += VecIO<OUT>::to_f32(g.e[3]);
+  }
+  O4 o;
+  o.e[0] = VecIO<OUT>::from_f32(r0);
+  o.e[1] = VecIO<OUT>::from_f32(r1);
+  o.e[2] = VecIO<OUT>::from_f32(r2);
+  o.e[3] = VecIO<OUT>::from_f32(r3);
+  *p = o;
+}
+
+template <typename OUT>
+__global__ void k_splitk_reduce(const float* __restrict__ ws, SplitDst<OUT> d,
+                                int z, int64_t n) {
   int64_t i = (int64_t)blockIdx.x * blockDim.x + threadIdx.x;
   int64_t stride = (int64_t)gridDim.x * blockDim.x;
   for (; i < n; i += stride) {
     float acc = 0.0f;
     for (int s = 0; s < z; ++s) acc += ws[(int64_t)s * n + i];
-    out[i] = VecIO<OUT>::from_f32(acc);
+    OUT* o = d.at(i);
+    if (d.acc) acc += VecIO<OUT>::to_f32(*o);
+    *o = VecIO<OUT>::from_f32(acc);
   }
 }
 
 template <typename OUT>
 __global__ void k_splitk_reduce4(const float4* __restrict__ ws,
-                                 OUT* __restrict__ out, int z, int64_t n4) {
+                                 SplitDst<OUT> d, int z, int64_t n4) {
   int64_t i = (int64_t)blockIdx.x * blockDim.x + threadIdx.x;
   int64_t stride = (int64_t)gridDim.x * blockDim.x;
   for (; i < n4; i += stride) {
@@ -1158,21 +1195,15 @@
       float4 v = ws[(int64_t)s * n4 + i];
       a0.x += v.x; a0.y += v.y; a0.z += v.z; a0.w += v.w;
     }
-    float r[4];
-    r[0] = (a0.x + a1.x) + (a2.x + a3.x);
-    r[1] = (a0.y + a1.y) + (a2.y + a3.y);
-    r[2] = (a0.z + a1.z) + (a2.z + a3.z);
-    r[3] = (a0.w + a1.w) + (a2.w + a3.w);
-    struct alignas(4 * sizeof(OUT)) O4 { OUT e[4]; } o;
-#pragma unroll
-    for (int j = 0; j < 4; ++j) o.e[j] = VecIO<OUT>::from_f32(r[j]);
-    ((O4*)out)[i] = o;
+    split_store4(d, i, (a0.x + a1.x) + (a2.x + a3.x),
+                 (a0.y + a1.y) + (a2.y + a3.y), (a0.z + a1.z) + (a2.z + a3.z),
+                 (a0.w + a1.w) + (a2.w + a3.w));
   }
 }
 
 template <typename OUT, int CPB>
-__global__ void k_splitk_fold(const float4* __restrict__ ws,
-                              OUT* __restrict__ out, int z, int64_t n4) {
+__global__ void k_splitk_fold(const float4* __restrict__ ws, SplitDst<OUT> d,
+                              int z, int64_t n4) {
   constexpr int RPB = 256 / CPB;
   __shared__ float4 sh[256];
   const int cl = threadIdx.x % CPB;
@@ -1197,22 +1228,17 @@
   }
   if (r == 0 && c < n4) {
     float4 m = sh[cl];
-    struct alignas(4 * sizeof(OUT)) O4 { OUT e[4]; } o;
-    o.e[0] = VecIO<OUT>::from_f32(m.x);
-    o.e[1] = VecIO<OUT>::from_f32(m.y);
-    o.e[2] = VecIO<OUT>::from_f32(m.z);
-    o.e[3] = VecIO<OUT>::from_f32(m.w);
-    ((O4*)out)[c] = o;
+    split_store4(d, c, m.x, m.y, m.z, m.w);
   }
 }
 
 template <typename OUT>
-static void splitk_fold_launch(const float4* ws, OUT* out, int z, int64_t n4,
-                               hipStream_t s, int64_t n4_shape) {
+static void splitk_fold_launch(const float4* ws, SplitDst<OUT> d, int z,
+                               int64_t n4, hipStream_t s, int64_t n4_shape) {
 #define FOLD_CASE(CPB)                                                    \
   hipLaunchKernelGGL((k_splitk_fold<OUT, CPB>),                           \
                      dim3((unsigned)((n4 + CPB - 1) / CPB)), dim3(256), 0, \
-                     s, ws, out, z, n4)
+                     s, ws, d, z, n4)
   if (n4_shape >= 128 * 32) FOLD_CASE(32);
   else if (n4_shape >= 128 * 16) FOLD_CASE(16);
   else if (n4_shape >= 128 * 8) FOLD_CASE(8);
@@ -1222,23 +1248,40 @@
 #undef FOLD_CASE
 }
 
+bool splitk_reduce_can_split(int64_t n, int64_t n0, const void* out0,
+                             const void* out1, DT out_dt) {
+  if ((n & 3) != 0) return true;
+  const uintptr_t al = (out_dt == DT::F32 ? 16 : 8) - 1;
+  return (n0 & 3) == 0 && ((uintptr_t)out0 & al) == 0 &&
+         ((uintptr_t)out1 & al) == 0;
+}
+
 void splitk_reduce_launch(const float* ws, void* out, DT out_dt, int z,
-                          int64_t n, hipStream_t s, int64_t n_shape) {
+                          int64_t n, hipStream_t s, int64_t n_shape,
+                          void* out1, int64_t n0, bool accumulate) {
   if (n_shape <= 0) n_shape = n;
+  if (!out1) n0 = n;
+  if (out1 && (n0 < 0 || n0 > n ||
+               !splitk_reduce_can_split(n, n0, out, out1, out_dt)))
+    throw std::invalid_argument(
+        "splitk_reduce_launch: the two destinations cannot be split here "
+        "(boundary or pointer off a group of 4); see splitk_reduce_can_split");
   dispatch_dt(out_dt, [&](auto tag) {
     using OUT = typename decltype(tag)::type;
+    const int acc = accumulate ? 1 : 0;
+    const SplitDst<OUT> d1{(OUT*)out, (OUT*)out1, n0, acc};
+    const SplitDst<OUT> d4{(OUT*)out, (OUT*)out1, n0 >> 2, acc};
     if ((n & 3) == 0 && (n_shape & 3) == 0 && n_shape < 4 * 32768 && z >= 8) {
-      splitk_fold_launch((const float4*)ws, (OUT*)out, z, n >> 2, s,
-                         n_shape >> 2);
+      splitk_fold_launch((const float4*)ws, d4, z, n >> 2, s, n_shape >> 2);
     } else if ((n & 3) == 0) {
       int64_t n4 = n >> 2;
       int blocks = (int)std::min<int64_t>((n4 + 255) / 256, (int64_t)2048);
       hipLaunchKernelGGL(k_splitk_reduce4<OUT>, dim3(blocks), dim3(256), 0, s,
-                         (const float4*)ws, (OUT*)out, z, n4);
+                         (const float4*)ws, d4, z, n4);
     } else {
       int blocks = (int)std::min<int64_t>((n + 255) / 256, (int64_t)2048);
       hipLaunchKernelGGL(k_splitk_reduce<OUT>, dim3(blocks), dim3(256), 0, s,
-                         ws, (OUT*)out, z, n);
+                         ws, d1, z, n);
     }
   });
 }
diff --git a/tnn_amd/csrc/kernels.h b/tnn_amd/csrc/kernels.h
--- a/tnn_amd/csrc/kernels.h
+++ b/tnn_amd/csrc/kernels.h
@@ -43,7 +43,8 @@
 void colsum_launch(DT dt, const void* x, void* out_f32, float* ws,
                    int rslices, int64_t rows, int64_t cols, hipStream_t s);
 void slab_fin_launch(const float* ws, float* out, int slices, int c2,
-                     hipStream_t s);
+                     hipStream_t s, float* d0 = nullptr, float* d1 = nullptr,
+                     bool accumulate = false);
 void cast_f32_launch(DT dt_out, const float* x, void* y, int64_t n,
                      hipStream_t s);
 
@@ -85,7 +86,11 @@
                     DT out_dt, float* ws, int z, const void* zero16, int M,
                     int N, int K, hipStream_t s);
 void splitk_reduce_launch(const float* ws, void* out, DT out_dt, int z,
-                          int64_t n, hipStream_t s, int64_t n_shape = 0);
+                          int64_t n, hipStream_t s, int64_t n_shape = 0,
+                          void* out1 = nullptr, int64_t n0 = 0,
+                          bool accumulate = false);
+bool splitk_reduce_can_split(int64_t n, int64_t n0, const void* out0,
+                             const void* out1, DT out_dt);
 void mfma_selftest_launch(const void* a_bf16, const void* b_bf16, float* d,
                           hipStream_t s);
 void mfma_selftest_f32_launch(const float* a, const float* b, float* d,
@@ -125,6 +130,7 @@
 bool conv2d_fwd_wants_db(DT dt, const void* x, const ConvShape& cs);
 void transpose_w_fwd_launch(DT dt, const void* w, void* w_t2, int KHW, int Cin,
                             int Cout, hipStream_t s);
+int conv2d_fwd_stats_rows(const ConvShape& cs);
 void conv2d_fwd_launch(DT dt, const void* x, const void* w, const void* w_t2,
                        const void* bias, void* y, const void* zero16,
                        float* stats, const ConvShape& cs, bool relu,
@@ -142,9 +148,14 @@
                                const ConvShape& cs);
 int conv2d_wgrad_zsplits(DT dt, const void* x, const void* dy,
                          const ConvShape& cs);
+struct WgradSink {
+  void* db_out = nullptr;
+  bool accumulate = false;
+};
 void conv2d_wgrad_launch(DT dt, const void* x, const void* dy, void* dw_out,
                          DT out_dt, float* ws, int z, const void* zero16,
-                         const ConvShape& cs, bool bias, hipStream_t s);
+                         const ConvShape& cs, bool bias, hipStream_t s,
+                         const WgradSink* sink = nullptr);
 void transpose_w_launch(DT dt, const void* w, void* w_t, int KH, int KW,
                         int Cin, int Cout, hipStream_t s);
 
@@ -156,6 +167,10 @@
                         float* invstd, float* rmean, float* rvar,
                         float momentum, int64_t rows, int cols, float eps,
                         hipStream_t s);
+void bn_finalize_fold_launch(const float* partials, int slices, float* mean,
+                             float* invstd, float* rmean, float* rvar,
+                             float momentum, int64_t rows, int cols, float eps,
+                             hipStream_t s);
 void bn_apply_launch(DT dt, const void* x, const float* mean,
                      const float* invstd, const float* gamma, const float* beta,
                      void* y, int64_t rows, int cols, bool relu, hipStream_t s);
@@ -173,7 +188,9 @@
 void bn_bwd_reduce_launch(DT dt, const void* x, const void* dy, const void* y_relu,
                           const float* mean, const float* invstd, float* sum_dy,
                           float* sum_dy_xhat, float* ws, int64_t rows, int cols,
-                          float dy_scale, hipStream_t s);
+                          float dy_scale, hipStream_t s,
+                          float* dgamma_out = nullptr,
+                          float* dbeta_out = nullptr, bool accumulate = false);
 void bn_bwd_apply_launch(DT dt, const void* x, const void* dy, const void* y_relu,
                          const float* mean, const float* invstd,
                          const float* gamma, const float* sum_dy,
diff --git a/tnn_amd/ops/functional.py b/tnn_amd/ops/functional.py
--- a/tnn_amd/ops/functional.py
+++ b/tnn_amd/ops/functional.py
@@ -41,6 +41,57 @@
     _graph_ctr = t
 
 
+class GradSinks:
+
+    def __init__(self, params=()):
+        self._buf = {}
+        self.written = set()
+        for p in params:
+            self.register(p, p.grad)
+
+    def register(self, param: torch.Tensor, buf: torch.Tensor):
+        if (buf is None or buf.shape != param.shape or buf.dtype != param.dtype
+                or buf.device != param.device or not buf.is_contiguous()):
+            raise ValueError("gradient sink must be a contiguous buffer of the "
+                             "parameter's shape, dtype and device")
+        self._buf[param.data_ptr()] = buf
+
+    def begin_step(self):
+        self.written.clear()
+
+    def get(self, key, like: Optional[torch.Tensor] = None):
+        buf = self._buf.get(key)
+        if buf is not None and like is not None and (
+                buf.shape != like.shape or buf.dtype != like.dtype):
+            return None
+        return buf
+
+    def claim(self, key) -> bool:
+        accumulate = key in self.written
+        self.written.add(key)
+        return accumulate
+
+
+_grad_sinks: Optional[GradSinks] = None
+
+
+def grad_sinks_enabled() -> bool:
+    import os
+    return os.environ.get("TNN_GRAD_SINK", "1") != "0"
+
+
+def set_grad_sinks(sinks: Optional[GradSinks]):
+    global _grad_sinks
+    _grad_sinks = sinks
+
+
+def _sink_key(t: Optional[torch.Tensor]):
+    if (_grad_sinks is None or t is None or not t.requires_grad
+            or not t.is_contiguous()):
+        return None
+    return t.data_ptr()
+
+
 def _draw_seed() -> int:
     if _graph_ctr is not None:
         import random
@@ -57,13 +108,15 @@
         Ci = x.shape[-1]
         V = 8 if x.dtype == torch.bfloat16 else 4
         ctx.cin = Ci
+        ctx.sink_keys = (_sink_key(w), _sink_key(bias))
         if Ci % V != 0 and Ci < V:
             x = F.pad(x, (0, V - Ci))
             w = F.pad(w, (0, 0, 0, V - Ci))
         ctx.want_stats = want_stats
         if want_stats:
-            y, stats = ext.conv2d_fwd_stats(x, w, bias, stride[0], stride[1],
-                                            padding[0], padding[1])
+            y, stats = ext.conv2d_fwd_partials(x, w, bias, stride[0],
+                                               stride[1], padding[0],
+                                               padding[1])
         else:
             y = ext.conv2d_fwd(x, w, bias, stride[0], stride[1], padding[0],
                                padding[1], fuse_relu)
@@ -72,11 +125,14 @@
         ctx.has_bias = bias is not None
         if want_stats:
             ctx.mark_non_differentiable(stats)
+            ctx.set_materialize_grads(False)
             return y, stats
         return y
 
     @staticmethod
     def backward(ctx, dy, *unused_stats_grad):
+        if dy is None:
+            return None, None, None, None, None, None, None
         x, w, y = ctx.saved_tensors
         ext = _C.ext()
         dy = dy.contiguous()
@@ -89,6 +145,10 @@
             if x.shape[-1] != ctx.cin:
                 dx = dx[..., :ctx.cin].contiguous()
         want_db = ctx.has_bias and ctx.needs_input_grad[2]
+        if ctx.needs_input_grad[1] and _grad_sinks is not None:
+            sunk = _Conv2dNHWC._wgrad_into_sinks(ctx, x, w, dy, want_db)
+            if sunk is not None:
+                return (dx,) + sunk + (None, None, None, None)
         if ctx.needs_input_grad[1]:
             args = (x, dy, w.shape[0], w.shape[1], ctx.stride[0],
                     ctx.stride[1], ctx.padding[0], ctx.padding[1],
@@ -104,6 +164,45 @@
         elif want_db:
             db = ext.colsum(dy.reshape(-1, dy.shape[-1]))
         return dx, dw, db, None, None, None, None
+
+    @staticmethod
+    def _wgrad_into_sinks(ctx, x, w, dy, want_db):
+        sinks = _grad_sinks
+        wkey, bkey = ctx.sink_keys
+        padded = x.shape[-1] != ctx.cin
+        dwbuf = dbbuf = None
+        if w.dtype not in (x.dtype, torch.float32):
+            return None
+        if not padded:
+            dwbuf = sinks.get(wkey, w)
+            if dwbuf is None:
+                return None
+        if want_db:
+            dbbuf = sinks.get(bkey, w[0, 0, 0])
+            if dbbuf is None:
+                return None
+        if dwbuf is None and dbbuf is None:
+            return None
+        if (dwbuf is not None and dbbuf is not None
+                and (wkey in sinks.written) != (bkey in sinks.written)):
+            return None
+        ext = _C.ext()
+        acc = False
+        if dwbuf is not None:
+            acc = sinks.claim(wkey)
+        if dbbuf is not None:
+            acc = sinks.claim(bkey)
+        dw = None
+        if padded:
+            dwbuf = (torch.zeros if acc else torch.empty)(
+                w.shape, dtype=w.dtype, device=w.device)
+            dw = dwbuf
+        ext.conv2d_wgrad_into(x, dy, w.shape[0], w.shape[1], ctx.stride[0],
+                              ctx.stride[1], ctx.padding[0], ctx.padding[1],
+                              dwbuf, dbbuf, acc)
+        if padded:
+            dw = dw[:, :, :ctx.cin].contiguous()
+        return dw, None
 
 
 def conv2d_nhwc(
@@ -137,6 +236,22 @@
 
 
 
+def _bn_sinks(ctx, x, dy) -> dict:
+    sinks = _grad_sinks
+    if sinks is None or not (ctx.needs_input_grad[1]
+                             and ctx.needs_input_grad[2]):
+        return {}
+    gkey, bkey = ctx.sink_keys
+    gbuf, bbuf = sinks.get(gkey), sinks.get(bkey)
+    if (gbuf is None or bbuf is None or gbuf.dtype != torch.float32
+            or bbuf.dtype != torch.float32
+            or (gkey in sinks.written) != (bkey in sinks.written)
+            or not _C.ext().bn_bwd_takes_sink(x, dy)):
+        return {}
+    sinks.claim(gkey)
+    return dict(dgamma_out=gbuf, dbeta_out=bbuf, accumulate=sinks.claim(bkey))
+
+
 class _BatchNormAct(torch.autograd.Function):
     @staticmethod
     def forward(ctx, x, gamma, beta, running_mean, running_var, momentum,
@@ -147,17 +262,26 @@
                                            dropout_p, seed, precomp, ctr)
         save_y = y if (relu or dropout_p > 0.0) else None
         ctx.save_for_backward(x, gamma, mean, invstd, save_y)
+        ctx.sink_keys = (_sink_key(gamma), _sink_key(beta))
         ctx.relu = relu or dropout_p > 0.0
         ctx.dy_scale = 1.0 / (1.0 - dropout_p) if dropout_p > 0.0 else 1.0
         ctx.mark_non_differentiable(mean, invstd)
+        ctx.set_materialize_grads(False)
         return y, mean, invstd
 
     @staticmethod
     def backward(ctx, dy, _dmean, _dinvstd):
+        if dy is None:
+            return (None,) * 12
         x, gamma, mean, invstd, y = ctx.saved_tensors
         ext = _C.ext()
-        dx, dgamma, dbeta = ext.bn_bwd(x, dy.contiguous(), gamma, mean, invstd,
-                                       y if ctx.relu else None, ctx.dy_scale)
+        dy = dy.contiguous()
+        sink = _bn_sinks(ctx, x, dy)
+        dx, dgamma, dbeta = ext.bn_bwd(x, dy, gamma, mean, invstd,
+                                       y if ctx.relu else None, ctx.dy_scale,
+                                       **sink)
+        if sink:
+            dgamma = dbeta = None
         return (dx, dgamma, dbeta, None, None, None, None, None, None, None,
                 None, None)
 
@@ -173,6 +297,7 @@
                                            dropout_p, seed, precomp, ctr)
         save_y = y if (relu or dropout_p > 0.0) else None
         ctx.save_for_backward(x, gamma, mean, invstd, save_y)
+        ctx.sink_keys = (_sink_key(gamma), _sink_key(beta))
         ctx.relu = relu or dropout_p > 0.0
         ctx.dy_scale = 1.0 / (1.0 - dropout_p) if dropout_p > 0.0 else 1.0
         ctx.mark_non_differentiable(mean, invstd)
@@ -188,9 +313,13 @@
                     None, None, None)
         if dres is not None:
             dres = dres.contiguous()
-        dx, dgamma, dbeta = ext.bn_bwd(x, dy.contiguous(), gamma, mean,
-                                       invstd, y if ctx.relu else None,
-                                       ctx.dy_scale, resid=dres)
+        dy = dy.contiguous()
+        sink = _bn_sinks(ctx, x, dy)
+        dx, dgamma, dbeta = ext.bn_bwd(x, dy, gamma, mean, invstd,
+                                       y if ctx.relu else None, ctx.dy_scale,
+                                       resid=dres, **sink)
+        if sink:
+            dgamma = dbeta = None
         return (dx, dgamma, dbeta, None, None, None, None, None, None, None,
                 None, None)
 
diff --git a/tnn_amd/utils/graphstep.py b/tnn_amd/utils/graphstep.py
--- a/tnn_amd/utils/graphstep.py
+++ b/tnn_amd/utils/graphstep.py
@@ -31,11 +31,27 @@
         return self.static_out
 
 
+ZERO_MERGE_GAP = 16384
+
+
+def unwritten_runs(layout, written, merge_gap: int = ZERO_MERGE_GAP):
+    runs = []
+    for key, off, numel in layout:
+        if key in written or numel == 0:
+            continue
+        if runs and off - runs[-1][1] <= merge_gap:
+            runs[-1][1] = off + numel
+        else:
+            runs.append([off, off + numel])
+    return [(a, b) for a, b in runs]
+
+
 class GraphedTrainStep:
 
     def __init__(self, model, criterion, optimizer, example_x, example_y,
                  warmup: int = 3):
-        from ..ops.functional import set_graph_seed_ctr
+        from ..ops.functional import (GradSinks, grad_sinks_enabled,
+                                      set_graph_seed_ctr, set_grad_sinks)
         assert example_x.is_cuda
         self.model, self.criterion, self.optimizer = model, criterion, optimizer
         self.static_x = example_x.clone()
@@ -52,15 +68,24 @@
         for prm in optimizer.params:
             groups.setdefault(prm.dtype, []).append(prm)
         self._grad_slabs = []
+        self._slab_layout = []
         for dt, ps in groups.items():
             slab = torch.zeros(sum(pp.numel() for pp in ps), dtype=dt,
                                device=dev)
             off = 0
+            layout = []
             for pp in ps:
                 pp.grad = slab[off:off + pp.numel()].view_as(pp)
+                layout.append((pp.data_ptr(), off, pp.numel()))
                 off += pp.numel()
             self._grad_slabs.append(slab)
+            self._slab_layout.append(layout)
+        self._sinks = (GradSinks(optimizer.params) if grad_sinks_enabled()
+                       else None)
+        self._sink_written = None
+        self._zero_views = None
         set_graph_seed_ctr(self.step_ctr)
+        set_grad_sinks(self._sinks)
         try:
             stream = torch.cuda.Stream()
             stream.wait_stream(torch.cuda.current_stream())
@@ -73,14 +98,34 @@
                 self.static_loss = self._step_body()
         finally:
             set_graph_seed_ctr(None)
+            set_grad_sinks(None)
 
     def _step_body(self):
         self.step_ctr.add_(1)
-        for slab in self._grad_slabs:
-            slab.zero_()
+        if self._sinks is not None:
+            self._sinks.begin_step()
+        if self._zero_views is None:
+            for slab in self._grad_slabs:
+                slab.zero_()
+        else:
+            for v in self._zero_views:
+                v.zero_()
         out = self.model(self.static_x)
         loss = self.criterion(out, self.static_y)
         loss.backward()
+        if self._sinks is not None:
+            written = frozenset(self._sinks.written)
+            if self._sink_written is None:
+                self._sink_written = written
+                self._zero_views = [
+                    slab[a:b]
+                    for slab, layout in zip(self._grad_slabs,
+                                            self._slab_layout)
+                    for a, b in unwritten_runs(layout, written)]
+            else:
+                assert written == self._sink_written, (
+                    "the gradient sinks wrote another set of parameters than "
+                    "in the first step; the zeroing plan no longer holds")
         self.optimizer.step()
         return loss
 
```
